# dylkot/cNMF

Measured on NVIDIA H100. Metric: NMF restarts/sec on NxG counts, K-sweep x100 seeds, 1/2/4/8 H100 vs sklearn CPU, higher is better.
Workload: dtype f32 (2-pass split-fp16 tensor-core products of group-normalised factors x exact integer counts, fp32 accumulate)

## Files before the change

cnmf_b200/_lib.py:

```python
import ctypes
import os

import numpy as np

_HERE = os.path.dirname(os.path.abspath(__file__))
LIB_PATH = os.path.join(_HERE, "libcnmf_b200.so")

SOLVER_MU, SOLVER_CD = 0, 1
PRECISION_FP32, PRECISION_TF32X3, PRECISION_TF32X3_GENERAL, PRECISION_F16X2, PRECISION_FP64 = 0, 1, 2, 3, 4
LOSS_FROBENIUS, LOSS_KULLBACK_LEIBLER, LOSS_ITAKURA_SAITO = 0, 1, 2
INIT_RANDOM, INIT_NNDSVD, INIT_NNDSVDA, INIT_NNDSVDAR = 0, 1, 2, 3
INIT_CODES = {"random": INIT_RANDOM, "nndsvd": INIT_NNDSVD, "nndsvda": INIT_NNDSVDA, "nndsvdar": INIT_NNDSVDAR}
MAX_COMPONENTS = 32


class CnmfError(RuntimeError):
    pass


class NmfParams(ctypes.Structure):
    _fields_ = [("solver", ctypes.c_int32), ("precision", ctypes.c_int32), ("max_iter", ctypes.c_int32),
                ("reserved", ctypes.c_int32), ("tol", ctypes.c_double),
                ("l1_reg_W", ctypes.c_double), ("l2_reg_W", ctypes.c_double),
                ("l1_reg_H", ctypes.c_double), ("l2_reg_H", ctypes.c_double),
                ("beta_loss", ctypes.c_int32), ("reserved2", ctypes.c_int32)]


UNIT_SOLVER_NONE = -1
UNIT_PIECES_NONE, UNIT_PIECES_TF32, UNIT_PIECES_F16 = 0, 1, 2
UNIT_GRAM_NONE, UNIT_GRAM_FUSED, UNIT_GRAM_STANDALONE = 0, 1, 2


class UpdateStepArgs(ctypes.Structure):
    _fields_ = [("n_slots", ctypes.c_int32), ("n_rids", ctypes.c_int32),
                ("ks", ctypes.c_void_p), ("rids", ctypes.c_void_p), ("done", ctypes.c_void_p),
                ("n", ctypes.c_int32), ("cpb_tiles", ctypes.c_int32), ("solver", ctypes.c_int32),
                ("pieces", ctypes.c_int32), ("gram", ctypes.c_int32), ("want_scalar", ctypes.c_int32),
                ("nsplit", ctypes.c_int32), ("l1", ctypes.c_float), ("l2", ctypes.c_float),
                ("F", ctypes.c_void_p), ("num", ctypes.c_void_p), ("gram_in", ctypes.c_void_p),
                ("piece_scale", ctypes.c_void_p), ("pieces_hi", ctypes.c_void_p), ("pieces_lo", ctypes.c_void_p),
                ("tile_scale", ctypes.c_void_p), ("gram_out", ctypes.c_void_p), ("scal_out", ctypes.c_void_p)]


UNIT_BETA_UPDATE, UNIT_BETA_DIVERGENCE = 0, 1
UNIT_SIDE_W, UNIT_SIDE_H = 0, 1


class BetaStepArgs(ctypes.Structure):
    _fields_ = [("n_slots", ctypes.c_int32), ("n_rids", ctypes.c_int32),
                ("ks", ctypes.c_void_p), ("rids", ctypes.c_void_p), ("done", ctypes.c_void_p),
                ("op", ctypes.c_int32), ("side", ctypes.c_int32), ("loss", ctypes.c_int32),
                ("n_items", ctypes.c_int32), ("n_contract", ctypes.c_int32), ("l1", ctypes.c_float), ("l2", ctypes.c_float),
                ("D", ctypes.c_void_p), ("F_own", ctypes.c_void_p), ("F_other", ctypes.c_void_p),
                ("oth_sum", ctypes.c_void_p), ("last", ctypes.c_void_p), ("totals", ctypes.c_void_p)]


_c = ctypes
_vp, _i, _ll, _d = _c.c_void_p, _c.c_int, _c.c_longlong, _c.c_double
_pp = _c.POINTER

SIGNATURES = {
    "cnmf_abi_version": (_i, []),
    "cnmf_last_error": (_c.c_char_p, []),
    "cnmf_create": (_i, [_pp(_vp), _i]),
    "cnmf_destroy": (_i, [_vp]),
    "cnmf_launch_count": (_ll, [_vp]),
    "cnmf_mem_info": (_i, [_vp, _pp(_ll), _pp(_ll), _pp(_ll)]),
    "cnmf_solve_bytes_per_row": (_ll, [_vp]),
    "cnmf_profile_enable": (_i, [_vp, _i]),
    "cnmf_profile_get": (_i, [_vp, _pp(_d), _pp(_ll), _pp(_d)]),
    "cnmf_profile_get_class": (_i, [_vp, _i, _pp(_d), _pp(_ll), _pp(_d)]),
    "cnmf_last_timing": (_i, [_vp, _pp(_d), _pp(_d), _pp(_d), _pp(_d)]),
    "cnmf_dataset_create": (_i, [_vp, _vp, _i, _i, _ll, _i, _i, _vp, _pp(_vp)]),
    "cnmf_dataset_create_csc": (_i, [_vp, _i, _i, _ll, _vp, _vp, _vp, _i, _vp, _pp(_vp)]),
    "cnmf_dataset_dense_bytes": (_i, [_i, _i, _i, _pp(_ll)]),
    "cnmf_dataset_from_columns": (_i, [_vp, _vp, _vp, _i, _vp, _pp(_vp)]),
    "cnmf_dataset_destroy": (_i, [_vp]),
    "cnmf_dataset_shape": (_i, [_vp, _pp(_i), _pp(_i)]),
    "cnmf_dataset_ld": (_i, [_vp, _pp(_i), _pp(_i)]),
    "cnmf_dataset_is_exact": (_i, [_vp]),
    "cnmf_dataset_sums": (_i, [_vp, _pp(_d), _pp(_d)]),
    "cnmf_dataset_min": (_i, [_vp, _pp(_c.c_float), _vp]),
    "cnmf_dataset_col_stats": (_i, [_vp, _vp, _vp, _vp]),
    "cnmf_dataset_row_sums": (_i, [_vp, _vp, _vp]),
    "cnmf_dataset_scaled_col_stats": (_i, [_vp, _vp, _vp, _vp, _vp]),
    "cnmf_dataset_scale_rows": (_i, [_vp, _vp, _vp, _pp(_vp)]),
    "cnmf_dataset_tpm_stats": (_i, [_vp, _d, _vp, _vp, _vp, _vp]),
    "cnmf_random_init_host": (_i, [_c.c_uint32, _d, _i, _i, _i, _vp, _ll, _vp, _ll]),
    "cnmf_random_init_dev": (_i, [_vp, _i, _vp, _vp, _vp, _vp, _vp]),
    "cnmf_nndsvd_init_dev": (_i, [_vp, _i, _vp, _vp, _i, _vp, _vp, _vp]),
    "cnmf_nndsvd_chunk_limit": (_i, [_vp, _i]),
    "cnmf_nndsvd_gemm_host": (_i, [_vp, _i, _i, _vp, _vp, _vp]),
    "cnmf_dataset_create_f64": (_i, [_vp, _vp, _i, _i, _ll, _i, _vp, _pp(_vp)]),
    "cnmf_dataset_from_columns_f64": (_i, [_vp, _vp, _vp, _i, _vp, _pp(_vp)]),
    "cnmf_factorize_f64": (_i, [_vp, _i, _vp, _vp, _pp(NmfParams), _vp, _vp, _vp, _vp, _vp]),
    "cnmf_factorize_init_f64": (_i, [_vp, _i, _vp, _vp, _vp, _pp(NmfParams), _vp, _vp, _vp, _vp, _vp]),
    "cnmf_refit_f64": (_i, [_vp, _i, _i, _vp, _pp(NmfParams), _vp, _pp(_c.c_int32), _pp(_d), _vp]),
    "cnmf_project_rows_f64": (_i, [_vp, _i, _vp, _vp, _vp]),
    "cnmf_factorize": (_i, [_vp, _i, _vp, _vp, _pp(NmfParams), _vp, _vp, _vp, _vp, _vp]),
    "cnmf_factorize_seeds_dev": (_i, [_vp, _i, _vp, _vp, _pp(NmfParams), _vp, _ll, _vp, _vp, _vp]),
    "cnmf_allgather_spectra": (_i, [_vp, _vp, _ll, _ll, _vp, _vp]),
    "cnmf_comm_unique_id": (_i, [_vp]),
    "cnmf_comm_create": (_i, [_vp, _vp, _i, _i, _pp(_vp)]),
    "cnmf_comm_destroy": (_i, [_vp]),
    "cnmf_factorize_init": (_i, [_vp, _i, _vp, _vp, _vp, _pp(NmfParams), _vp, _vp, _vp, _vp, _vp]),
    "cnmf_factorize_dev": (_i, [_vp, _i, _vp, _vp, _vp, _pp(NmfParams), _vp, _vp, _vp, _vp]),
    "cnmf_refit": (_i, [_vp, _i, _i, _vp, _pp(NmfParams), _vp, _pp(_c.c_int32), _pp(_d), _vp]),
    "cnmf_project_rows": (_i, [_vp, _i, _vp, _vp, _vp]),
    "cnmf_gemm_abt_host": (_i, [_vp, _i, _vp, _vp, _i, _i, _i, _i, _i, _vp, _vp, _vp, _i, _pp(_c.c_float), _vp]),
    "cnmf_update_step_host": (_i, [_vp, _pp(UpdateStepArgs), _vp]),
    "cnmf_beta_step_host": (_i, [_vp, _pp(BetaStepArgs), _vp]),
    "cnmf_l2_normalize_rows": (_i, [_vp, _vp, _i, _i, _i, _vp]),
    "cnmf_local_density": (_i, [_vp, _vp, _i, _i, _i, _i, _vp, _vp, _vp]),
    "cnmf_col_stats_dev": (_i, [_vp, _vp, _i, _i, _i, _vp, _vp, _vp]),
    "cnmf_gather_rows": (_i, [_vp, _vp, _i, _vp, _i, _i, _vp, _i, _vp]),
    "cnmf_sq_dists_to_rows": (_i, [_vp, _vp, _i, _i, _i, _vp, _i, _vp, _vp]),
    "cnmf_kmeans_step": (_i, [_vp, _vp, _i, _i, _i, _i, _vp, _vp, _vp, _vp, _vp, _vp, _vp, _vp, _pp(_c.c_int32), _pp(_c.c_int32), _pp(_d), _vp]),
    "cnmf_kmeans_fit": (_i, [_vp, _vp, _i, _i, _i, _i, _i, _i, _d, _vp, _vp, _i, _vp, _vp, _vp, _pp(_c.c_int32), _vp]),
    "cnmf_kmeans_assign": (_i, [_vp, _vp, _i, _i, _i, _vp, _i, _vp, _vp, _vp, _vp, _vp, _vp, _vp]),
    "cnmf_cluster_dist_sums": (_i, [_vp, _vp, _i, _i, _i, _vp, _i, _vp, _vp]),
    "cnmf_cluster_median": (_i, [_vp, _vp, _i, _i, _i, _vp, _i, _vp, _i, _vp]),
    "cnmf_l2_normalize_rows_f64": (_i, [_vp, _vp, _i, _i, _i, _vp]),
    "cnmf_local_density_f64": (_i, [_vp, _vp, _i, _i, _i, _i, _vp, _vp, _vp]),
    "cnmf_col_stats_dev_f64": (_i, [_vp, _vp, _i, _i, _i, _vp, _vp, _vp]),
    "cnmf_gather_rows_f64": (_i, [_vp, _vp, _i, _vp, _i, _i, _vp, _i, _vp]),
    "cnmf_sq_dists_to_rows_f64": (_i, [_vp, _vp, _i, _i, _i, _vp, _i, _vp, _vp]),
    "cnmf_kmeans_step_f64": (_i, [_vp, _vp, _i, _i, _i, _i, _vp, _vp, _vp, _vp, _vp, _vp, _pp(_c.c_int32), _pp(_c.c_int32), _pp(_d), _vp]),
    "cnmf_kmeans_fit_f64": (_i, [_vp, _vp, _i, _i, _i, _i, _i, _i, _d, _vp, _vp, _i, _vp, _vp, _vp, _pp(_c.c_int32), _vp]),
    "cnmf_kmeans_assign_f64": (_i, [_vp, _vp, _i, _i, _i, _vp, _i, _vp, _vp, _vp, _vp, _vp, _vp, _vp]),
    "cnmf_cluster_dist_sums_f64": (_i, [_vp, _vp, _i, _i, _i, _vp, _i, _vp, _vp]),
    "cnmf_cluster_median_f64": (_i, [_vp, _vp, _i, _i, _i, _vp, _i, _vp, _i, _vp]),
}

_lib = None


ABI_VERSION = 14


def load():
    global _lib
    if _lib is not None:
        return _lib
    if not os.path.exists(LIB_PATH):
        raise CnmfError(
            "libcnmf_b200.so not found at %s -- build it with `python -m cnmf_b200.build` "
            "(cnmf_b200 has no CPU / PyTorch fallback)" % LIB_PATH)
    lib = ctypes.CDLL(LIB_PATH)
    for name, (res, args) in SIGNATURES.items():
        fn = getattr(lib, name)
        fn.restype = res
        fn.argtypes = args
    if lib.cnmf_abi_version() != ABI_VERSION:
        raise CnmfError("libcnmf_b200.so ABI version mismatch")
    _lib = lib
    return lib


def check(rc):
    if rc != 0:
        msg = load().cnmf_last_error()
        raise CnmfError("cnmf_b200 error %d: %s" % (rc, msg.decode() if msg else "?"))


def ptr(a):
    if a is None:
        return None
    assert a.flags["C_CONTIGUOUS"]
    return a.ctypes.data_as(ctypes.c_void_p)


def f32c(a):
    return np.ascontiguousarray(a, dtype=np.float32)


def f64c(a):
    return np.ascontiguousarray(a, dtype=np.float64)
```

cnmf_b200/csrc/capi_refit.cu:

```cuda
#include <algorithm>
#include <chrono>
#include <cmath>
#include <cstring>
#include <vector>

#include "engine.h"
#include "gemm.h"
#include "nmf_kernels.cuh"

using namespace cnmf;

namespace {

__global__ void fill_kernel(float* p, float v, int rows, int n, int ld) {
  const long long total = (long long)rows * n;
  for (long long i = blockIdx.x * (long long)blockDim.x + threadIdx.x; i < total; i += (long long)gridDim.x * blockDim.x)
    p[(i / n) * ld + (i % n)] = v;
}

template <typename T>
__global__ void col_stats_kernel(const T* __restrict__ X, int rows, int cols, int ld,
                                 const double* __restrict__ row_scale, double* __restrict__ part) {
  const int c = blockIdx.x * blockDim.x + threadIdx.x;
  if (c >= cols) return;
  const int per = (rows + gridDim.y - 1) / gridDim.y;
  const int r0 = blockIdx.y * per, r1 = min(rows, r0 + per);
  double s = 0.0, q = 0.0;
  for (int r = r0; r < r1; ++r) {
    double v = X[(long long)r * ld + c];
    if (row_scale) v *= row_scale[r];
    s += v;
    q += v * v;
  }
  part[((long long)blockIdx.y * 2) * cols + c] = s;
  part[((long long)blockIdx.y * 2 + 1) * cols + c] = q;
}

__global__ void gather_cols_div_kernel(const double* __restrict__ src, int rows, int ld_src, const int* __restrict__ cols,
                                       const double* __restrict__ divisor, int n_cols, double* __restrict__ dst,
                                       int ld_dst) {
  const int c = blockIdx.x * blockDim.x + threadIdx.x;
  if (c >= n_cols) return;
  const int sc = cols[c];
  const double f = divisor[c];
  for (int r = blockIdx.y; r < rows; r += gridDim.y)
    dst[(long long)r * ld_dst + c] = __ddiv_rn(src[(long long)r * ld_src + sc], f);
}

__global__ void transpose64_kernel(const double* __restrict__ F, int k, int n, int ld, double* __restrict__ out) {
  const long long total = (long long)n * k;
  for (long long i = blockIdx.x * (long long)blockDim.x + threadIdx.x; i < total; i += (long long)gridDim.x * blockDim.x)
    out[i] = F[(i % k) * ld + i / k];
}

__global__ void col_stats_reduce_kernel(const double* __restrict__ part, int strips, int cols, double* __restrict__ out) {
  const int c = blockIdx.x * blockDim.x + threadIdx.x;
  if (c >= cols) return;
  double s = 0.0, q = 0.0;
  for (int y = 0; y < strips; ++y) {
    s += part[((long long)y * 2) * cols + c];
    q += part[((long long)y * 2 + 1) * cols + c];
  }
  out[c] = s;
  out[cols + c] = q;
}

__global__ void row_sums_kernel(const float* __restrict__ X, int rows, int cols, int ld, double* __restrict__ out) {
  const int r = (blockIdx.x * blockDim.x + threadIdx.x) >> 5, lane = threadIdx.x & 31;
  if (r >= rows) return;
  const float* row = X + (long long)r * ld;
  double s = 0.0;
  for (int c = lane; c < cols; c += 32) s += (double)row[c];
  s = warp_sum(s);
  if (lane == 0) out[r] = s;
}

__global__ void scale_rows_kernel(const float* __restrict__ src, int rows, int cols, int ld, const float* __restrict__ rs,
                                  float* __restrict__ dst) {
  const long long total = (long long)rows * (ld / 4);
  for (long long i = blockIdx.x * (long long)blockDim.x + threadIdx.x; i < total; i += (long long)gridDim.x * blockDim.x) {
    const int r = (int)(i / (ld / 4));
    float4 v = reinterpret_cast<const float4*>(src)[i];
    const float f = rs[r];
    v.x *= f; v.y *= f; v.z *= f; v.w *= f;
    reinterpret_cast<float4*>(dst)[i] = v;
  }
}

__global__ void combine_scale_kernel(const float* __restrict__ scale, const float* __restrict__ src_cs,
                                     const int* __restrict__ cols, int n, int n_pad, float* __restrict__ out) {
  const int c = blockIdx.x * blockDim.x + threadIdx.x;
  if (c >= n_pad) return;
  out[c] = (c < n) ? scale[c] * (src_cs ? src_cs[cols[c]] : 1.f) : 0.f;
}

__global__ void gather_cols_kernel(const float* __restrict__ src, int rows, int ld_src, const int* __restrict__ cols,
                                   const float* __restrict__ scale, int n_cols, float* __restrict__ dst, int ld_dst) {
  const int c = blockIdx.x * blockDim.x + threadIdx.x;
  if (c >= n_cols) return;
  const int sc = cols[c];
  const float f = scale[c];
  for (int r = blockIdx.y; r < rows; r += gridDim.y) dst[(long long)r * ld_dst + c] = src[(long long)r * ld_src + sc] * f;
}

}

extern "C" {

static void finish_col_stats(double n, int n_cols, double* mean_host, double* var_host) {
  for (int c = 0; c < n_cols; ++c) {
    const double m = mean_host[c] / n;
    mean_host[c] = m;
    var_host[c] = std::max(var_host[c] / n - m * m, 0.0);
  }
}

static int col_stats_impl(cnmf_dataset_t d, const double* row_scale_host, double* mean_host, double* var_host, void* stream) {
  CNMF_REQUIRE(d && mean_host && var_host, "col_stats: NULL argument");
  cnmf_handle_s* h = d->h;
  cudaStream_t s = as_stream(stream);
  CNMF_CUDA_CHECK(cudaSetDevice(h->device));
  if (row_scale_host) CNMF_TRY(require_dense(d, "scaled_col_stats"));
  const bool f64 = d->precision == CNMF_PRECISION_FP64;
  double* buf = d->col_sums;
  if (!d->sparse) {
    const int strips = std::max(1, std::min(64, d->n_rows / 64));
    double* part = static_cast<double*>(h->dev_buf("colstats.part", sizeof(double) * 2 * (size_t)strips * d->n_cols));
    buf = static_cast<double*>(h->dev_buf("colstats", sizeof(double) * 2 * d->n_cols));
    double* d_rs = nullptr;
    if (row_scale_host) {
      d_rs = static_cast<double*>(h->dev_buf("colstats.rs", sizeof(double) * d->n_rows));
      if (!d_rs) return -2;
      CNMF_CUDA_CHECK(cudaMemcpyAsync(d_rs, row_scale_host, sizeof(double) * d->n_rows, cudaMemcpyHostToDevice, s));
    }
    if (!part || !buf) return -2;
    dim3 grid((d->n_cols + 127) / 128, strips);
    if (f64) col_stats_kernel<<<grid, 128, 0, s>>>(d->X64, d->n_rows, d->n_cols, d->ld_c, d_rs, part);
    else col_stats_kernel<<<grid, 128, 0, s>>>(d->X, d->n_rows, d->n_cols, d->ld_c, d_rs, part);
    col_stats_reduce_kernel<<<(d->n_cols + 127) / 128, 128, 0, s>>>(part, strips, d->n_cols, buf);
    CNMF_CUDA_CHECK(cudaGetLastError());
    h->launches += 2;
  }
  CNMF_CUDA_CHECK(cudaMemcpyAsync(mean_host, buf, sizeof(double) * d->n_cols, cudaMemcpyDeviceToHost, s));
  CNMF_CUDA_CHECK(cudaMemcpyAsync(var_host, buf + d->n_cols, sizeof(double) * d->n_cols, cudaMemcpyDeviceToHost, s));
  CNMF_CUDA_CHECK(cudaStreamSynchronize(s));
  finish_col_stats(d->n_rows, d->n_cols, mean_host, var_host);
  return 0;
}

int cnmf_dataset_col_stats(cnmf_dataset_t d, double* mean_host, double* var_host, void* stream) {
  return col_stats_impl(d, nullptr, mean_host, var_host, stream);
}

int cnmf_dataset_scaled_col_stats(cnmf_dataset_t d, const double* row_scale_host, double* mean_host, double* var_host,
                                  void* stream) {
  CNMF_REQUIRE(row_scale_host, "scaled_col_stats: NULL row scale");
  return col_stats_impl(d, row_scale_host, mean_host, var_host, stream);
}

int cnmf_dataset_row_sums(cnmf_dataset_t d, double* row_sums_host, void* stream) {
  CNMF_REQUIRE(d && row_sums_host, "row_sums: NULL argument");
  CNMF_TRY(require_dense(d, "row_sums"));
  cnmf_handle_s* h = d->h;
  cudaStream_t s = as_stream(stream);
  CNMF_CUDA_CHECK(cudaSetDevice(h->device));
  double* buf = static_cast<double*>(h->dev_buf("rowsums", sizeof(double) * d->n_rows));
  if (!buf) return -2;
  row_sums_kernel<<<(d->n_rows + 7) / 8, 256, 0, s>>>(d->X, d->n_rows, d->n_cols, d->ld_c, buf);
  CNMF_CUDA_CHECK(cudaGetLastError());
  h->launches += 1;
  CNMF_CUDA_CHECK(cudaMemcpyAsync(row_sums_host, buf, sizeof(double) * d->n_rows, cudaMemcpyDeviceToHost, s));
  CNMF_CUDA_CHECK(cudaStreamSynchronize(s));
  return 0;
}

int cnmf_dataset_tpm_stats(cnmf_dataset_t d, double target_sum, double* totals_host, double* mean_host,
                           double* var_host, void* stream) {
  CNMF_REQUIRE(d && totals_host && mean_host && var_host, "tpm_stats: NULL argument");
  if (!d->sparse) {
    set_last_error("tpm_stats is implemented for sparse (CSC) datasets only: a dense dataset gives the same numbers "
                   "through row_sums and scaled_col_stats");
    return -3;
  }
  cnmf_handle_s* h = d->h;
  cudaStream_t s = as_stream(stream);
  CNMF_CUDA_CHECK(cudaSetDevice(h->device));
  double* tot = static_cast<double*>(h->dev_buf("rowsums", sizeof(double) * d->n_rows));
  double* sums = static_cast<double*>(h->dev_buf("colstats", sizeof(double) * 2 * d->n_cols));
  if (!tot || !sums) return -2;
  CNMF_TRY(csc_tpm_sums(d, target_sum, tot, sums, s));
  CNMF_CUDA_CHECK(cudaMemcpyAsync(totals_host, tot, sizeof(double) * d->n_rows, cudaMemcpyDeviceToHost, s));
  CNMF_CUDA_CHECK(cudaMemcpyAsync(mean_host, sums, sizeof(double) * d->n_cols, cudaMemcpyDeviceToHost, s));
  CNMF_CUDA_CHECK(cudaMemcpyAsync(var_host, sums + d->n_cols, sizeof(double) * d->n_cols, cudaMemcpyDeviceToHost, s));
  CNMF_CUDA_CHECK(cudaStreamSynchronize(s));
  finish_col_stats(d->n_rows, d->n_cols, mean_host, var_host);
  return 0;
}

int cnmf_dataset_from_columns(cnmf_dataset_t src, const int32_t* cols_host, const float* col_scale_host, int n_cols,
                              void* stream, cnmf_dataset_t* out) {
  CNMF_REQUIRE(src && cols_host && col_scale_host && out && n_cols > 0, "dataset_from_columns: bad arguments");
  CNMF_TRY(require_f32(src, "dataset_from_columns"));
  for (int c = 0; c < n_cols; ++c)
    CNMF_REQUIRE(cols_host[c] >= 0 && cols_host[c] < src->n_cols, "dataset_from_columns: column index out of range");
  cnmf_handle_s* h = src->h;
  cudaStream_t s = as_stream(stream);
  CNMF_CUDA_CHECK(cudaSetDevice(h->device));
  int* d_cols = static_cast<int*>(h->dev_buf("fromcols.idx", sizeof(int) * n_cols));
  float* d_scale = static_cast<float*>(h->dev_buf("fromcols.scale", sizeof(float) * n_cols));
  if (!d_cols || !d_scale) return -2;
  CNMF_CUDA_CHECK(cudaMemcpyAsync(d_cols, cols_host, sizeof(int) * n_cols, cudaMemcpyHostToDevice, s));
  CNMF_CUDA_CHECK(cudaMemcpyAsync(d_scale, col_scale_host, sizeof(float) * n_cols, cudaMemcpyHostToDevice, s));
  auto* d = new cnmf_dataset_s(h, src->n_rows, n_cols, src->precision);
  int rc = dataset_alloc(d, &d->X, (size_t)d->n_rows * d->ld_c);
  if (rc == 0) {
    cudaError_t e = cudaMemsetAsync(d->X, 0, (size_t)d->n_rows * d->ld_c * sizeof(float), s);
    if (e != cudaSuccess) rc = -2;
  }
  if (rc == 0 && src->sparse) {
    rc = csc_gather_cols(src, d_cols, d_scale, n_cols, d->X, d->ld_c, s);
  } else if (rc == 0) {
    dim3 grid((n_cols + 127) / 128, std::min(d->n_rows, 16384));
    gather_cols_kernel<<<grid, 128, 0, s>>>(src->X, d->n_rows, src->ld_c, d_cols, d_scale, n_cols, d->X, d->ld_c);
    h->launches += 1;
    if (cudaGetLastError() != cudaSuccess) rc = -2;
  }
  const bool exact = form_exact(src->form);
  if (rc == 0 && exact) {
    rc = dataset_alloc(d, &d->col_scale, (size_t)d->ld_c);
    if (rc == 0) {
      combine_scale_kernel<<<(d->ld_c + 255) / 256, 256, 0, s>>>(d_scale, src->col_scale, d_cols, n_cols, d->ld_c, d->col_scale);
      h->launches += 1;
      if (cudaGetLastError() != cudaSuccess) rc = -2;
    }
    if (rc == 0 && src->row_scale) {
      rc = dataset_alloc(d, &d->row_scale, (size_t)d->ld_r);
      if (rc == 0 && cudaMemcpyAsync(d->row_scale, src->row_scale, sizeof(float) * d->ld_r, cudaMemcpyDeviceToDevice, s) != cudaSuccess)
        rc = -2;
    }
  }
  if (rc == 0) rc = dataset_finish(d, s, exact);
  if (rc != 0) {
    cnmf_dataset_destroy(d);
    return rc;
  }
  *out = d;
  return 0;
}

int cnmf_dataset_scale_rows(cnmf_dataset_t src, const float* row_scale_host, void* stream, cnmf_dataset_t* out) {
  CNMF_REQUIRE(src && row_scale_host && out, "dataset_scale_rows: bad arguments");
  CNMF_TRY(require_dense(src, "scale_rows"));
  cnmf_handle_s* h = src->h;
  cudaStream_t s = as_stream(stream);
  CNMF_CUDA_CHECK(cudaSetDevice(h->device));
  float* d_rs = static_cast<float*>(h->dev_buf("scalerows.rs", sizeof(float) * src->n_rows));
  if (!d_rs) return -2;
  CNMF_CUDA_CHECK(cudaMemcpyAsync(d_rs, row_scale_host, sizeof(float) * src->n_rows, cudaMemcpyHostToDevice, s));
  auto* d = new cnmf_dataset_s(h, src->n_rows, src->n_cols, src->precision);
  int rc = dataset_alloc(d, &d->X, (size_t)d->n_rows * d->ld_c);
  if (rc == 0) {
    scale_rows_kernel<<<NUM_SMS * 8, 256, 0, s>>>(src->X, d->n_rows, d->n_cols, d->ld_c, d_rs, d->X);
    h->launches += 1;
    if (cudaGetLastError() != cudaSuccess) rc = -2;
  }
  if (rc == 0) rc = dataset_finish(d, s);
  if (rc != 0) {
    cnmf_dataset_destroy(d);
    return rc;
  }
  *out = d;
  return 0;
}

int cnmf_refit(cnmf_dataset_t d, int transposed, int k, const float* fixed_host, const cnmf_nmf_params* p,
               float* out_host, int32_t* n_iter_host, double* err_host, void* stream) {
  CNMF_REQUIRE(d && fixed_host && p && out_host, "refit: NULL argument");
  CNMF_TRY(require_f32(d, "refit"));
  CNMF_TRY(check_params_precision(d, p));
  CNMF_REQUIRE(k >= 1 && k <= KMAX, "refit: n_components must be in [1, 32] on the CUDA path");
  if (d->sparse && !transposed) CNMF_TRY(require_dense(d, "refit with transposed = 0"));
  if (d->sparse && p->beta_loss != CNMF_LOSS_FROBENIUS) CNMF_TRY(require_dense(d, "refit with a KL / IS beta_loss"));
  const auto t_enter = std::chrono::steady_clock::now();
  cnmf_handle_s* h = d->h;
  cudaStream_t s = as_stream(stream);
  CNMF_CUDA_CHECK(cudaSetDevice(h->device));
  if (p->beta_loss != CNMF_LOSS_FROBENIUS) CNMF_TRY(dataset_ensure_full_transpose(d, s));
  const DataView v = make_view(d, transposed != 0);

  const size_t nr = (size_t)k * v.ld_r, nc = (size_t)k * v.ld_c;
  float* Fr = static_cast<float*>(h->dev_buf("refit.Fr", nr * 4));
  float* Fc = static_cast<float*>(h->dev_buf("refit.Fc", nc * 4));
  if (!Fr || !Fc) return -2;
  CNMF_CUDA_CHECK(cudaMemsetAsync(Fr, 0, nr * 4, s));
  CNMF_CUDA_CHECK(cudaMemsetAsync(Fc, 0, nc * 4, s));
  CNMF_CUDA_CHECK(cudaMemcpy2DAsync(Fc, (size_t)v.ld_c * 4, fixed_host, (size_t)v.n_c * 4, (size_t)v.n_c * 4, k,
                                    cudaMemcpyHostToDevice, s));
  if (p->solver == CNMF_SOLVER_MU) {
    const double mean = v.sum / ((double)v.n_r * (double)v.n_c);
    fill_kernel<<<NUM_SMS * 4, 256, 0, s>>>(Fr, (float)std::sqrt(mean / k), k, v.n_r, v.ld_r);
    CNMF_CUDA_CHECK(cudaGetLastError());
    h->launches += 1;
  }
  SolveIO io;
  io.R = 1;
  io.ks = {k};
  io.Fr = Fr;
  io.Fc = Fc;
  io.update_cols = false;
  if (d->sparse) {
    const int kp = round_up(k, 4);
    float* U = static_cast<float*>(h->dev_buf("refit.U", (size_t)v.n_c * kp * 4));
    float* NUM = static_cast<float*>(h->dev_buf("refit.NUM", nr * 4));
    if (!U || !NUM) return -2;
    CNMF_CUDA_CHECK(cudaMemsetAsync(NUM, 0, nr * 4, s));
    CNMF_TRY(stage_rows(h, Fc, k, v.n_c, v.ld_c, kp, U, s));
    CNMF_TRY(csc_project(d, U, k, kp, NUM, v.ld_r, s));
    io.num_rows = NUM;
  }
  auto t_solve = std::chrono::steady_clock::now();
  if (h->profile) {
    CNMF_CUDA_CHECK(cudaStreamSynchronize(s));
    h->t_h2d_ms = std::chrono::duration<double, std::milli>(t_solve - t_enter).count();
    t_solve = std::chrono::steady_clock::now();
  }
  CNMF_TRY(solve_batched(h, v, io, *p, s));
  if (h->profile) h->t_solve_ms = std::chrono::duration<double, std::milli>(std::chrono::steady_clock::now() - t_solve).count();

  float* T = static_cast<float*>(h->dev_buf("refit.T", (size_t)v.n_r * k * 4));
  float* T_host = static_cast<float*>(h->host_buf("refit.T_host", (size_t)v.n_r * k * 4));
  if (!T || !T_host) return -2;
  CNMF_TRY(launch_transpose(Fr, k, v.n_r, v.ld_r, T, nullptr, nullptr, k, s));
  h->launches += 1;
  CNMF_CUDA_CHECK(cudaMemcpyAsync(T_host, T, (size_t)v.n_r * k * 4, cudaMemcpyDeviceToHost, s));
  CNMF_CUDA_CHECK(cudaStreamSynchronize(s));
  std::memcpy(out_host, T_host, (size_t)v.n_r * k * 4);
  if (n_iter_host) *n_iter_host = io.n_iter[0];
  if (err_host) *err_host = io.err[0];
  return 0;
}

int cnmf_project_rows(cnmf_dataset_t d, int k, const float* Ut_host, float* out_host, void* stream) {
  CNMF_REQUIRE(d && Ut_host && out_host && k >= 1, "project_rows: bad arguments");
  CNMF_TRY(require_f32(d, "project_rows"));
  cnmf_handle_s* h = d->h;
  cudaStream_t s = as_stream(stream);
  CNMF_CUDA_CHECK(cudaSetDevice(h->device));
  if (d->sparse) {
    CNMF_REQUIRE(k <= KMAX, "project_rows: k must be <= 32 on a sparse dataset");
    const int kp = round_up(k, 4);
    float* Ut = static_cast<float*>(h->dev_buf("proj.Ut", (size_t)k * d->n_rows * 4));
    float* U = static_cast<float*>(h->dev_buf("proj.U", (size_t)d->n_rows * kp * 4));
    float* C = static_cast<float*>(h->dev_buf("proj.C", (size_t)k * d->ld_c * 4));
    if (!Ut || !U || !C) return -2;
    CNMF_CUDA_CHECK(cudaMemcpyAsync(Ut, Ut_host, (size_t)k * d->n_rows * 4, cudaMemcpyHostToDevice, s));
    CNMF_TRY(stage_rows(h, Ut, k, d->n_rows, d->n_rows, kp, U, s));
    CNMF_TRY(csc_project(d, U, k, kp, C, d->ld_c, s));
    CNMF_CUDA_CHECK(cudaMemcpy2DAsync(out_host, (size_t)d->n_cols * 4, C, (size_t)d->ld_c * 4, (size_t)d->n_cols * 4, k,
                                      cudaMemcpyDeviceToHost, s));
    CNMF_CUDA_CHECK(cudaStreamSynchronize(s));
    return 0;
  }
  const DataView v = make_view(d, false);
  const size_t nr = (size_t)k * d->ld_r;
  float* A = static_cast<float*>(h->dev_buf("proj.A", nr * 4));
  float *A_hi = nullptr, *A_lo = nullptr, *A_rs = nullptr;
  if (!A) return -2;
  CNMF_CUDA_CHECK(cudaMemsetAsync(A, 0, nr * 4, s));
  CNMF_CUDA_CHECK(cudaMemcpy2DAsync(A, (size_t)d->ld_r * 4, Ut_host, (size_t)d->n_rows * 4, (size_t)d->n_rows * 4, k,
                                    cudaMemcpyHostToDevice, s));
  if (v.form != Form::FP32) {
    A_hi = static_cast<float*>(h->dev_buf("proj.A_hi", nr * 4));
    A_lo = static_cast<float*>(h->dev_buf("proj.A_lo", nr * 4));
    if (!A_hi || !A_lo) return -2;
    if (v.form == Form::F16_EXACT) {
      A_rs = static_cast<float*>(h->dev_buf("proj.A_rs", sizeof(float) * (size_t)k * ((d->ld_r + 511) / 512)));
      if (!A_rs) return -2;
    }
    CNMF_TRY(make_pieces(v.form, A, k, d->n_rows, d->ld_r, v.scale_r, A_hi, A_lo, A_rs, s));
    h->launches += 1;
  }
  GemmArgs g{};
  g.M = k; g.N = d->n_cols; g.Kd = d->n_rows;
  g.lda = d->ld_r; g.ldb = d->ld_r; g.ldc = d->ld_c;
  int splits = 1;
  {
    const int tiles = ((k + 127) / 128) * ((d->n_cols + 255) / 256);
    if (tiles < 2 * h->sm_count) splits = (2 * h->sm_count + tiles - 1) / tiles;
    splits = std::min(splits, std::max(1, ((d->n_rows + 31) / 32) / 8));
    splits = std::min(splits, 32);
    splits = gemm_effective_splits(d->n_rows, splits, v.form == Form::F16_EXACT ? 1 : 0);
  }
  g.splits = g.splits_effective = splits;
  g.c_split_stride = (long long)k * d->ld_c;
  float* C = static_cast<float*>(h->dev_buf("proj.C", (size_t)splits * k * d->ld_c * 4));
  if (!C) return -2;
  g.C = C;
  CNMF_TRY(form_gemm(v.form, g, A, A_hi, A_lo, A_rs, v.B_cols, v.scale_c, s));
  h->launches += 1;
  std::vector<float> tmp((size_t)splits * k * d->ld_c);
  CNMF_CUDA_CHECK(cudaMemcpyAsync(tmp.data(), C, tmp.size() * 4, cudaMemcpyDeviceToHost, s));
  CNMF_CUDA_CHECK(cudaStreamSynchronize(s));
  for (int c = 0; c < k; ++c)
    for (int j = 0; j < d->n_cols; ++j) {
      double a = 0.0;
      for (int z = 0; z < splits; ++z) a += tmp[(size_t)z * k * d->ld_c + (size_t)c * d->ld_c + j];
      out_host[(size_t)c * d->n_cols + j] = (float)a;
    }
  return 0;
}

int cnmf_dataset_from_columns_f64(cnmf_dataset_t src, const int32_t* cols_host, const double* divisor_host, int n_cols,
                                  void* stream, cnmf_dataset_t* out) {
  CNMF_REQUIRE(src && cols_host && divisor_host && out && n_cols > 0, "dataset_from_columns_f64: bad arguments");
  CNMF_TRY(require_f64(src, "dataset_from_columns"));
  for (int c = 0; c < n_cols; ++c)
    CNMF_REQUIRE(cols_host[c] >= 0 && cols_host[c] < src->n_cols, "dataset_from_columns_f64: column index out of range");
  cnmf_handle_s* h = src->h;
  cudaStream_t s = as_stream(stream);
  CNMF_CUDA_CHECK(cudaSetDevice(h->device));
  int* d_cols = static_cast<int*>(h->dev_buf("fromcols.idx", sizeof(int) * n_cols));
  double* d_div = static_cast<double*>(h->dev_buf("fromcols.div64", sizeof(double) * n_cols));
  if (!d_cols || !d_div) return -2;
  CNMF_CUDA_CHECK(cudaMemcpyAsync(d_cols, cols_host, sizeof(int) * n_cols, cudaMemcpyHostToDevice, s));
  CNMF_CUDA_CHECK(cudaMemcpyAsync(d_div, divisor_host, sizeof(double) * n_cols, cudaMemcpyHostToDevice, s));
  auto* d = new cnmf_dataset_s(h, src->n_rows, n_cols, CNMF_PRECISION_FP64);
  d->form = Form::FP64;
  const size_t nx = (size_t)d->n_rows * d->ld_c;
  float* buf = nullptr;
  int rc = dataset_alloc(d, &buf, 2 * nx);
  if (rc == 0) {
    d->X64 = reinterpret_cast<double*>(buf);
    if (cudaMemsetAsync(d->X64, 0, nx * sizeof(double), s) != cudaSuccess) rc = -2;
  }
  if (rc == 0) {
    dim3 grid((n_cols + 127) / 128, std::min(d->n_rows, 16384));
    gather_cols_div_kernel<<<grid, 128, 0, s>>>(src->X64, d->n_rows, src->ld_c, d_cols, d_div, n_cols, d->X64, d->ld_c);
    h->launches += 1;
    if (cudaGetLastError() != cudaSuccess) rc = -2;
  }
  double sums[2] = {0.0, 0.0};
  if (rc == 0) rc = matrix_sums_f64(h, d->X64, d->n_rows, d->n_cols, d->ld_c, sums, s);
  if (rc != 0) {
    cnmf_dataset_destroy(d);
    return rc;
  }
  d->sum = sums[0];
  d->sum_sq = sums[1];
  *out = d;
  return 0;
}

int cnmf_refit_f64(cnmf_dataset_t d, int transposed, int k, const double* fixed_host, const cnmf_nmf_params* p,
                   double* out_host, int32_t* n_iter_host, double* err_host, void* stream) {
  CNMF_REQUIRE(d && fixed_host && p && out_host, "refit_f64: NULL argument");
  CNMF_TRY(require_f64(d, "refit"));
  CNMF_TRY(check_params_precision(d, p));
  CNMF_REQUIRE(k >= 1 && k <= KMAX, "refit_f64: n_components must be in [1, 32] on the CUDA path");
  if (p->beta_loss != CNMF_LOSS_FROBENIUS) {
    set_last_error("cnmf_refit_f64: float64 datasets support beta_loss = frobenius only");
    return -3;
  }
  cnmf_handle_s* h = d->h;
  cudaStream_t s = as_stream(stream);
  CNMF_CUDA_CHECK(cudaSetDevice(h->device));
  const DataView v = make_view(d, transposed != 0);
  const size_t nr = (size_t)k * v.ld_r, nc = (size_t)k * v.ld_c;
  double* Fr = static_cast<double*>(h->dev_buf("refit.Fr64", nr * 8));
  double* Fc = static_cast<double*>(h->dev_buf("refit.Fc64", nc * 8));
  double* T = static_cast<double*>(h->dev_buf("refit.T64", (size_t)v.n_r * k * 8));
  if (!Fr || !Fc || !T) return -2;
  CNMF_CUDA_CHECK(cudaMemsetAsync(Fr, 0, nr * 8, s));
  CNMF_CUDA_CHECK(cudaMemsetAsync(Fc, 0, nc * 8, s));
  CNMF_CUDA_CHECK(cudaMemcpy2DAsync(Fc, (size_t)v.ld_c * 8, fixed_host, (size_t)v.n_c * 8, (size_t)v.n_c * 8, k,
                                    cudaMemcpyHostToDevice, s));
  if (p->solver == CNMF_SOLVER_MU) {
    const double mean = v.sum / ((double)v.n_r * (double)v.n_c);
    CNMF_TRY(fill_f64(Fr, std::sqrt(mean / k), k, v.n_r, v.ld_r, s));
    h->launches += 1;
  }
  SolveIO io;
  io.R = 1;
  io.ks = {k};
  io.Fr64 = Fr;
  io.Fc64 = Fc;
  io.update_cols = false;
  CNMF_TRY(solve_batched(h, v, io, *p, s));
  transpose64_kernel<<<NUM_SMS * 4, 256, 0, s>>>(Fr, k, v.n_r, v.ld_r, T);
  CNMF_CUDA_CHECK(cudaGetLastError());
  h->launches += 1;
  CNMF_CUDA_CHECK(cudaMemcpyAsync(out_host, T, (size_t)v.n_r * k * 8, cudaMemcpyDeviceToHost, s));
  CNMF_CUDA_CHECK(cudaStreamSynchronize(s));
  if (n_iter_host) *n_iter_host = io.n_iter[0];
  if (err_host) *err_host = io.err[0];
  return 0;
}

int cnmf_project_rows_f64(cnmf_dataset_t d, int k, const double* Ut_host, double* out_host, void* stream) {
  CNMF_REQUIRE(d && Ut_host && out_host && k >= 1, "project_rows_f64: bad arguments");
  CNMF_TRY(require_f64(d, "project_rows"));
  cnmf_handle_s* h = d->h;
  cudaStream_t s = as_stream(stream);
  CNMF_CUDA_CHECK(cudaSetDevice(h->device));
  const size_t na = (size_t)k * d->ld_r, nc = (size_t)k * d->ld_c;
  double* A = static_cast<double*>(h->dev_buf("proj.A64", na * 8));
  double* C = static_cast<double*>(h->dev_buf("proj.C64", nc * 8));
  if (!A || !C) return -2;
  CNMF_CUDA_CHECK(cudaMemsetAsync(A, 0, na * 8, s));
  CNMF_CUDA_CHECK(cudaMemcpy2DAsync(A, (size_t)d->ld_r * 8, Ut_host, (size_t)d->n_rows * 8, (size_t)d->n_rows * 8, k,
                                    cudaMemcpyHostToDevice, s));
  h->launches += 1;
  CNMF_TRY(launch_gemm_f64(A, d->ld_r, k, d->X64, d->n_rows, d->n_cols, d->ld_c, true, C, d->ld_c, s));
  CNMF_CUDA_CHECK(cudaMemcpy2DAsync(out_host, (size_t)d->n_cols * 8, C, (size_t)d->ld_c * 8, (size_t)d->n_cols * 8, k,
                                    cudaMemcpyDeviceToHost, s));
  CNMF_CUDA_CHECK(cudaStreamSynchronize(s));
  return 0;
}

int cnmf_gemm_abt_host(cnmf_handle_t h, int precision, const float* A, const float* B, int M, int N, int Kd, int splits,
                       int b_exact, const float* k_scale, const float* out_col_scale, float* C, int reps, float* ms_out,
                       void* stream) {
  CNMF_REQUIRE(h && A && B && C && M > 0 && N > 0 && Kd > 0, "gemm_abt_host: bad arguments");
  const bool f16 = precision == CNMF_PRECISION_F16X2;
  CNMF_REQUIRE(!b_exact || f16 || precision == CNMF_PRECISION_TF32X3, "gemm_abt_host: b_exact needs tf32x3 or f16x2");
  const bool exact = f16 || b_exact;
  CNMF_REQUIRE(exact || (!k_scale && !out_col_scale), "gemm_abt_host: k_scale / out_col_scale need an exact form");
  const Form form = f16 ? Form::F16_EXACT
                  : precision != CNMF_PRECISION_TF32X3 ? Form::FP32
                  : b_exact ? Form::TF32_EXACT : Form::TF32;
  cudaStream_t s = as_stream(stream);
  CNMF_CUDA_CHECK(cudaSetDevice(h->device));
  const int lda = pad_ld(Kd), ldc = pad_ld(N);
  const size_t na = (size_t)M * lda, nb = (size_t)N * lda;
  float* dA = static_cast<float*>(h->dev_buf("gemmtest.A", na * 4));
  float* dB = static_cast<float*>(h->dev_buf("gemmtest.B", nb * 4));
  float* dAh = static_cast<float*>(h->dev_buf("gemmtest.Ah", na * 4));
  float* dAl = static_cast<float*>(h->dev_buf("gemmtest.Al", na * 4));
  float* dBh = static_cast<float*>(h->dev_buf("gemmtest.Bh", nb * 4));
  float* dBl = static_cast<float*>(h->dev_buf("gemmtest.Bl", nb * 4));
  const int se = gemm_effective_splits(Kd, splits, f16 ? 1 : 0);
  float* dC = static_cast<float*>(h->dev_buf("gemmtest.C", (size_t)se * M * ldc * 4));
  float* dRs = static_cast<float*>(h->dev_buf("gemmtest.rs", sizeof(float) * (size_t)M * ((lda + 511) / 512)));
  if (!dA || !dB || !dAh || !dAl || !dBh || !dBl || !dC || !dRs) return -2;
  CNMF_CUDA_CHECK(cudaMemsetAsync(dA, 0, na * 4, s));
  CNMF_CUDA_CHECK(cudaMemsetAsync(dB, 0, nb * 4, s));
  CNMF_CUDA_CHECK(cudaMemcpy2DAsync(dA, (size_t)lda * 4, A, (size_t)Kd * 4, (size_t)Kd * 4, M, cudaMemcpyHostToDevice, s));
  CNMF_CUDA_CHECK(cudaMemcpy2DAsync(dB, (size_t)lda * 4, B, (size_t)Kd * 4, (size_t)Kd * 4, N, cudaMemcpyHostToDevice, s));
  float* dKs = nullptr;
  float* dCs = nullptr;
  if (k_scale) {
    dKs = static_cast<float*>(h->dev_buf("gemmtest.kscale", (size_t)lda * 4));
    if (!dKs) return -2;
    CNMF_CUDA_CHECK(cudaMemsetAsync(dKs, 0, (size_t)lda * 4, s));
    CNMF_CUDA_CHECK(cudaMemcpyAsync(dKs, k_scale, (size_t)Kd * 4, cudaMemcpyHostToDevice, s));
  }
  if (out_col_scale) {
    dCs = static_cast<float*>(h->dev_buf("gemmtest.cscale", (size_t)ldc * 4));
    if (!dCs) return -2;
    CNMF_CUDA_CHECK(cudaMemsetAsync(dCs, 0, (size_t)ldc * 4, s));
    CNMF_CUDA_CHECK(cudaMemcpyAsync(dCs, out_col_scale, (size_t)N * 4, cudaMemcpyHostToDevice, s));
  }
  if (f16) CNMF_TRY(launch_to_half(dB, dBh, (long long)nb, s));
  else if (form != Form::FP32) CNMF_TRY(launch_split_tf32(dB, dBh, dBl, (long long)nb, s));
  CNMF_TRY(make_pieces(form, dA, M, Kd, lda, dKs, dAh, dAl, dRs, s));
  CNMF_CUDA_CHECK(cudaMemsetAsync(dC, 0xff, (size_t)se * M * ldc * 4, s));
  GemmArgs g{};
  g.M = M; g.N = N; g.Kd = Kd; g.lda = lda; g.ldb = lda; g.ldc = ldc;
  g.C = dC; g.c_split_stride = (long long)M * ldc; g.splits = splits; g.splits_effective = se;
  const Operand Bop{dB, dBh, dBl, N, Kd, lda};
  cudaEvent_t e0, e1;
  CNMF_CUDA_CHECK(cudaEventCreate(&e0));
  CNMF_CUDA_CHECK(cudaEventCreate(&e1));
  if (reps < 1) reps = 1;
  int rc = form_gemm(form, g, dA, dAh, dAl, dRs, Bop, dCs, s);
  if (rc == 0 && reps > 1) {
    cudaEventRecord(e0, s);
    for (int i = 0; i < reps && rc == 0; ++i) rc = form_gemm(form, g, dA, dAh, dAl, dRs, Bop, dCs, s);
    cudaEventRecord(e1, s);
  }
  h->launches += reps;
  if (rc != 0) return rc;
  std::vector<float> tmp((size_t)se * M * ldc);
  CNMF_CUDA_CHECK(cudaMemcpyAsync(tmp.data(), dC, tmp.size() * 4, cudaMemcpyDeviceToHost, s));
  CNMF_CUDA_CHECK(cudaStreamSynchronize(s));
  if (ms_out) {
    float ms = 0.f;
    if (reps > 1) cudaEventElapsedTime(&ms, e0, e1);
    *ms_out = reps > 1 ? ms / reps : 0.f;
  }
  cudaEventDestroy(e0);
  cudaEventDestroy(e1);
  for (int m = 0; m < M; ++m)
    for (int n = 0; n < N; ++n) {
      double a = 0.0;
      for (int z = 0; z < se; ++z) a += tmp[(size_t)z * M * ldc + (size_t)m * ldc + n];
      C[(size_t)m * N + n] = (float)a;
    }
  return 0;
}

}
```

cnmf_b200/csrc/gemm.h:

```cpp
#pragma once
#include <cuda_runtime.h>

namespace cnmf {

struct GemmArgs {
  const float* A_hi;
  const float* A_lo;
  const float* B_hi;
  const float* B_lo;
  float* C;
  int M, N, Kd;
  int lda, ldb, ldc;
  long long c_split_stride;
  int splits;
  int splits_effective;
  int b_exact;
  const float* out_col_scale;
  int f16;
  const float* a_tile_scale;
  int a_tiles;
};

int gemm_effective_splits(int Kd, int splits, int f16 = 0);

int gemm_fixed_splits(int Kd, int f16 = 0);

int gemm_tf32x3(const GemmArgs& g, cudaStream_t stream);

int gemm_fp32_simt(const GemmArgs& g, cudaStream_t stream);

}
```

cnmf_b200/csrc/gemm_tf32x3.cu:

```cuda
#include <cuda.h>
#include <cuda_runtime.h>
#include <cstdint>
#include <cstdio>
#include <algorithm>
#include <map>
#include <mutex>
#include <tuple>

#include "common.cuh"
#include "gemm.h"

namespace cnmf {

namespace {

constexpr int BN = 128;
constexpr int BK = 32;
constexpr long long WAIT_TIMEOUT_CYCLES = 4000000000LL;

template <int BM>
constexpr int num_threads() { return 128 * (1 + BM / 64); }

template <int BM, int STAGES, bool BEXACT>
struct SmemLayout {
  static constexpr int A_BYTES = BM * BK * 4;
  static constexpr int B_BYTES = BN * BK * 4;
  static constexpr int STAGE_BYTES = 2 * A_BYTES + (BEXACT ? 1 : 2) * B_BYTES;
  static constexpr int BAR_OFFSET = STAGES * STAGE_BYTES;
  static constexpr int TOTAL = BAR_OFFSET + 3 * STAGES * 8;
  static constexpr int DYN_BYTES = TOTAL + 1024;
  static_assert(DYN_BYTES <= 227 * 1024, "pipeline stages do not fit the shared memory of an SM");
};

__device__ __forceinline__ void mbar_init(uint32_t bar, uint32_t count) {
  asm volatile("mbarrier.init.shared::cta.b64 [%0], %1;" ::"r"(bar), "r"(count) : "memory");
}
__device__ __forceinline__ void mbar_arrive_expect_tx(uint32_t bar, uint32_t bytes) {
  asm volatile("mbarrier.arrive.expect_tx.shared::cta.b64 _, [%0], %1;" ::"r"(bar), "r"(bytes) : "memory");
}
__device__ __forceinline__ void mbar_arrive(uint32_t bar) {
  asm volatile("mbarrier.arrive.shared::cta.b64 _, [%0];" ::"r"(bar) : "memory");
}
__device__ __forceinline__ bool mbar_try_wait(uint32_t bar, uint32_t parity) {
  uint32_t ok;
  asm volatile(
      "{\n\t.reg .pred p;\n\t"
      "mbarrier.try_wait.parity.shared::cta.b64 p, [%1], %2;\n\t"
      "selp.u32 %0, 1, 0, p;\n\t}"
      : "=r"(ok)
      : "r"(bar), "r"(parity)
      : "memory");
  return ok != 0;
}
template <bool TRAP>
__device__ __forceinline__ void mbar_wait(uint32_t bar, uint32_t parity) {
  if (mbar_try_wait(bar, parity)) return;
  const long long t0 = clock64();
  while (!mbar_try_wait(bar, parity)) {
    if (TRAP && clock64() - t0 > WAIT_TIMEOUT_CYCLES) __trap();
  }
}
__device__ __forceinline__ void tma_load_2d(uint32_t dst, const CUtensorMap* map, uint32_t bar, int c0, int c1) {
  asm volatile(
      "cp.async.bulk.tensor.2d.shared::cluster.global.mbarrier::complete_tx::bytes [%0], [%1, {%3, %4}], [%2];"
      ::"r"(dst), "l"(reinterpret_cast<uint64_t>(map)), "r"(bar), "r"(c0), "r"(c1)
      : "memory");
}
__device__ __forceinline__ void tma_load_2d_multicast(uint32_t dst, const CUtensorMap* map, uint32_t bar, int c0, int c1,
                                                      uint16_t mask) {
  asm volatile(
      "cp.async.bulk.tensor.2d.shared::cluster.global.mbarrier::complete_tx::bytes.multicast::cluster"
      " [%0], [%1, {%3, %4}], [%2], %5;"
      ::"r"(dst), "l"(reinterpret_cast<uint64_t>(map)), "r"(bar), "r"(c0), "r"(c1), "h"(mask)
      : "memory");
}

__device__ __forceinline__ void mbar_arrive_remote(uint32_t bar, uint32_t rank) {
  asm volatile(
      "{\n\t.reg .b32 remote;\n\t"
      "mapa.shared::cluster.u32 remote, %0, %1;\n\t"
      "mbarrier.arrive.shared::cluster.b64 _, [remote];\n\t}"
      ::"r"(bar), "r"(rank)
      : "memory");
}
__device__ __forceinline__ void cluster_sync() {
  asm volatile("barrier.cluster.arrive.release;\n\tbarrier.cluster.wait.acquire;" ::: "memory");
}

__device__ __forceinline__ uint64_t make_smem_desc(uint32_t smem_addr) {
  uint64_t d = 0;
  d |= static_cast<uint64_t>((smem_addr & 0x3FFFFu) >> 4);
  d |= static_cast<uint64_t>(1) << 16;
  d |= static_cast<uint64_t>(1024 >> 4) << 32;
  d |= static_cast<uint64_t>(1) << 62;
  return d;
}

__device__ __forceinline__ void named_bar_sync(uint32_t id, uint32_t count) {
  asm volatile("bar.sync %0, %1;" ::"r"(id), "r"(count) : "memory");
}
__device__ __forceinline__ void named_bar_arrive(uint32_t id, uint32_t count) {
  asm volatile("bar.arrive %0, %1;" ::"r"(id), "r"(count) : "memory");
}

template <int N>
__device__ __forceinline__ void setmaxnreg_dec() { asm volatile("setmaxnreg.dec.sync.aligned.u32 %0;" ::"n"(N)); }
template <int N>
__device__ __forceinline__ void setmaxnreg_inc() { asm volatile("setmaxnreg.inc.sync.aligned.u32 %0;" ::"n"(N)); }

__device__ __forceinline__ void wgmma_fence() { asm volatile("wgmma.fence.sync.aligned;" ::: "memory"); }
__device__ __forceinline__ void wgmma_commit() { asm volatile("wgmma.commit_group.sync.aligned;" ::: "memory"); }
template <int N>
__device__ __forceinline__ void wgmma_wait() { asm volatile("wgmma.wait_group.sync.aligned %0;" ::"n"(N) : "memory"); }

template <bool F16>
__device__ __forceinline__ void wgmma_m64n128(float (&d)[64], uint64_t adesc, uint64_t bdesc, uint32_t acc) {
  if constexpr (F16) {
    asm volatile(
      "{\n\t.reg .pred p;\n\t"
      "setp.ne.b32 p, %66, 0;\n\t"
      "wgmma.mma_async.sync.aligned.m64n128k16.f32.f16.f16 {"
      "%0, %1, %2, %3, %4, %5, %6, %7, %8, %9, %10, %11, %12, %13, %14, %15, "
      "%16, %17, %18, %19, %20, %21, %22, %23, %24, %25, %26, %27, %28, %29, %30, %31, "
      "%32, %33, %34, %35, %36, %37, %38, %39, %40, %41, %42, %43, %44, %45, %46, %47, "
      "%48, %49, %50, %51, %52, %53, %54, %55, %56, %57, %58, %59, %60, %61, %62, %63 "
      "}, %64, %65, p, 1, 1, 0, 0;\n\t}"
      : "+f"(d[0]), "+f"(d[1]), "+f"(d[2]), "+f"(d[3]), "+f"(d[4]), "+f"(d[5]), "+f"(d[6]), "+f"(d[7]),
        "+f"(d[8]), "+f"(d[9]), "+f"(d[10]), "+f"(d[11]), "+f"(d[12]), "+f"(d[13]), "+f"(d[14]), "+f"(d[15]),
        "+f"(d[16]), "+f"(d[17]), "+f"(d[18]), "+f"(d[19]), "+f"(d[20]), "+f"(d[21]), "+f"(d[22]), "+f"(d[23]),
        "+f"(d[24]), "+f"(d[25]), "+f"(d[26]), "+f"(d[27]), "+f"(d[28]), "+f"(d[29]), "+f"(d[30]), "+f"(d[31]),
        "+f"(d[32]), "+f"(d[33]), "+f"(d[34]), "+f"(d[35]), "+f"(d[36]), "+f"(d[37]), "+f"(d[38]), "+f"(d[39]),
        "+f"(d[40]), "+f"(d[41]), "+f"(d[42]), "+f"(d[43]), "+f"(d[44]), "+f"(d[45]), "+f"(d[46]), "+f"(d[47]),
        "+f"(d[48]), "+f"(d[49]), "+f"(d[50]), "+f"(d[51]), "+f"(d[52]), "+f"(d[53]), "+f"(d[54]), "+f"(d[55]),
        "+f"(d[56]), "+f"(d[57]), "+f"(d[58]), "+f"(d[59]), "+f"(d[60]), "+f"(d[61]), "+f"(d[62]), "+f"(d[63])
      : "l"(adesc), "l"(bdesc), "r"(acc));
  } else {
    asm volatile(
      "{\n\t.reg .pred p;\n\t"
      "setp.ne.b32 p, %66, 0;\n\t"
      "wgmma.mma_async.sync.aligned.m64n128k8.f32.tf32.tf32 {"
      "%0, %1, %2, %3, %4, %5, %6, %7, %8, %9, %10, %11, %12, %13, %14, %15, "
      "%16, %17, %18, %19, %20, %21, %22, %23, %24, %25, %26, %27, %28, %29, %30, %31, "
      "%32, %33, %34, %35, %36, %37, %38, %39, %40, %41, %42, %43, %44, %45, %46, %47, "
      "%48, %49, %50, %51, %52, %53, %54, %55, %56, %57, %58, %59, %60, %61, %62, %63 "
      "}, %64, %65, p, 1, 1;\n\t}"
      : "+f"(d[0]), "+f"(d[1]), "+f"(d[2]), "+f"(d[3]), "+f"(d[4]), "+f"(d[5]), "+f"(d[6]), "+f"(d[7]),
        "+f"(d[8]), "+f"(d[9]), "+f"(d[10]), "+f"(d[11]), "+f"(d[12]), "+f"(d[13]), "+f"(d[14]), "+f"(d[15]),
        "+f"(d[16]), "+f"(d[17]), "+f"(d[18]), "+f"(d[19]), "+f"(d[20]), "+f"(d[21]), "+f"(d[22]), "+f"(d[23]),
        "+f"(d[24]), "+f"(d[25]), "+f"(d[26]), "+f"(d[27]), "+f"(d[28]), "+f"(d[29]), "+f"(d[30]), "+f"(d[31]),
        "+f"(d[32]), "+f"(d[33]), "+f"(d[34]), "+f"(d[35]), "+f"(d[36]), "+f"(d[37]), "+f"(d[38]), "+f"(d[39]),
        "+f"(d[40]), "+f"(d[41]), "+f"(d[42]), "+f"(d[43]), "+f"(d[44]), "+f"(d[45]), "+f"(d[46]), "+f"(d[47]),
        "+f"(d[48]), "+f"(d[49]), "+f"(d[50]), "+f"(d[51]), "+f"(d[52]), "+f"(d[53]), "+f"(d[54]), "+f"(d[55]),
        "+f"(d[56]), "+f"(d[57]), "+f"(d[58]), "+f"(d[59]), "+f"(d[60]), "+f"(d[61]), "+f"(d[62]), "+f"(d[63])
      : "l"(adesc), "l"(bdesc), "r"(acc));
  }
}

struct TileOrder {
  int m_tiles, n_pairs, group, group_n;
};

__host__ __device__ __forceinline__ void decode_item(int w, const TileOrder& o, int& mt, int& np, int& z) {
  const int per_slice = o.m_tiles * o.n_pairs;
  z = w / per_slice;
  int r = w - z * per_slice;
  const int q_tiles = o.group_n ? o.n_pairs : o.m_tiles;
  const int p_tiles = o.group_n ? o.m_tiles : o.n_pairs;
  const int g0 = r / (o.group * p_tiles) * o.group;
  r -= g0 * p_tiles;
  const int gq = q_tiles - g0 < o.group ? q_tiles - g0 : o.group;
  const int p = r / gq, q = g0 + r % gq;
  mt = o.group_n ? p : q;
  np = o.group_n ? q : p;
}

template <int BM, int STAGES, bool BEXACT, bool F16>
__device__ __forceinline__ void
gemm_body(const CUtensorMap& tmA_hi, const CUtensorMap& tmA_lo, const CUtensorMap& tmB_hi, const CUtensorMap& tmB_lo,
          float* __restrict__ C, int M, int ldc, long long c_split_stride,
          const TileOrder& ord, int n_tiles, int splits, int total_kb, int kb_per_split, int chain_kb,
          const float* __restrict__ out_scale, const float* __restrict__ a_tile_scale, int a_tiles, int a_gshift) {
  static_assert(!F16 || BEXACT, "the fp16 path exists for exact integer B operands only");
  static_assert(BM == 128 || BM == 192, "two or three consumer warpgroups");
  constexpr int NC = BM / 64;
  constexpr int BKE = F16 ? 2 * BK : BK;
  constexpr int KSTEP_BYTES = 32;
  using L = SmemLayout<BM, STAGES, BEXACT>;
  extern __shared__ uint8_t smem_raw[];
  const uint32_t smem_base = (smem_u32(smem_raw) + 1023u) & ~1023u;

  const uint32_t bar_base = smem_base + L::BAR_OFFSET;
  auto full_bar = [&](int s) { return bar_base + 8u * s; };
  auto empty_bar = [&](int s) { return bar_base + 8u * (STAGES + s); };
  auto peer_free_bar = [&](int s) { return bar_base + 8u * (2 * STAGES + s); };

  const int wg = __shfl_sync(0xffffffffu, static_cast<int>(threadIdx.x >> 7), 0);
  const int warp = (threadIdx.x >> 5) & 3;
  const int lane = threadIdx.x & 31;
  const int rank = blockIdx.x & 1, cluster = blockIdx.x >> 1, clusters = gridDim.x >> 1;

  if (threadIdx.x == 0) {
    for (int s = 0; s < STAGES; ++s) {
      mbar_init(full_bar(s), 1);
      mbar_init(empty_bar(s), 4 * NC);
      mbar_init(peer_free_bar(s), 1);
    }
    asm volatile("fence.mbarrier_init.release.cluster;" ::: "memory");
  }
  cluster_sync();

  const int items = ord.m_tiles * ord.n_pairs * splits;

  constexpr bool REBALANCE = NC == 3;
  if (wg == 0) {
    if constexpr (REBALANCE) setmaxnreg_dec<32>();
    if (threadIdx.x == 0) {
      int stage = 0;
      uint32_t phase = 0;
      constexpr uint32_t stage_tx = static_cast<uint32_t>(L::STAGE_BYTES);
      constexpr uint32_t HALF_A = L::A_BYTES / 2;
      for (int w = cluster; w < items; w += clusters) {
        int mt, np, z;
        decode_item(w, ord, mt, np, z);
        const int nt = 2 * np + rank;
        const int kb0 = z * kb_per_split;
        const int kb1 = min(total_kb, kb0 + kb_per_split);
        for (int kb = kb0; kb < kb1; ++kb) {
          mbar_wait<true>(empty_bar(stage), phase ^ 1u);
          mbar_arrive_remote(peer_free_bar(stage), rank ^ 1);
          mbar_wait<true>(peer_free_bar(stage), phase);
          const uint32_t st = smem_base + stage * L::STAGE_BYTES;
          mbar_arrive_expect_tx(full_bar(stage), stage_tx);
          tma_load_2d_multicast(st + rank * HALF_A, &tmA_hi, full_bar(stage), kb * BKE, mt * BM + rank * (BM / 2), 0x3);
          tma_load_2d_multicast(st + L::A_BYTES + rank * HALF_A, &tmA_lo, full_bar(stage), kb * BKE,
                                mt * BM + rank * (BM / 2), 0x3);
          tma_load_2d(st + 2 * L::A_BYTES, &tmB_hi, full_bar(stage), kb * BKE, nt * BN);
          if constexpr (!BEXACT) tma_load_2d(st + 2 * L::A_BYTES + L::B_BYTES, &tmB_lo, full_bar(stage), kb * BKE, nt * BN);
          if (++stage == STAGES) { stage = 0; phase ^= 1u; }
        }
      }
      for (int s = 0; s < STAGES; ++s) {
        mbar_wait<true>(empty_bar(stage), phase ^ 1u);
        if (++stage == STAGES) { stage = 0; phase ^= 1u; }
      }
    }
  } else {
    if constexpr (REBALANCE) setmaxnreg_inc<160>();
    constexpr uint32_t TURN_BAR = 1, TURN_THREADS = 256;
    const int cw = wg - 1;
    const uint32_t a_off = static_cast<uint32_t>(cw * 64 * 128);
    const uint32_t next_bar = TURN_BAR + (cw + 1 == NC ? 0 : cw + 1);
    if (cw == NC - 1) named_bar_arrive(TURN_BAR, TURN_THREADS);
    int stage = 0;
    uint32_t phase = 0;
    for (int w = cluster; w < items; w += clusters) {
      int mt, np, z;
      decode_item(w, ord, mt, np, z);
      const int nt = 2 * np + rank;
      const int kb0 = z * kb_per_split;
      const int kb1 = min(total_kb, kb0 + kb_per_split);
      const int row0 = mt * BM + cw * 64 + warp * 16 + (lane >> 2);
      float acc[64];
#pragma unroll
      for (int i = 0; i < 64; ++i) acc[i] = 0.f;
      const float* sc_row0 = (F16 && a_tile_scale && row0 < M) ? a_tile_scale + static_cast<long long>(row0) * a_tiles : nullptr;
      const float* sc_row1 = (F16 && a_tile_scale && row0 + 8 < M) ? a_tile_scale + static_cast<long long>(row0 + 8) * a_tiles : nullptr;
      for (int c0 = kb0; c0 < kb1; c0 += chain_kb) {
        const int c1 = min(kb1, c0 + chain_kb);
        float d[64];
        int prev = -1;
        for (int kb = c0; kb < c1; ++kb) {
          mbar_wait<false>(full_bar(stage), phase);
          named_bar_sync(TURN_BAR + cw, TURN_THREADS);
          const uint32_t st = smem_base + stage * L::STAGE_BYTES;
          const uint64_t a_hi = make_smem_desc(st + a_off);
          const uint64_t a_lo = make_smem_desc(st + L::A_BYTES + a_off);
          const uint64_t b_hi = make_smem_desc(st + 2 * L::A_BYTES);
          const uint64_t b_lo = make_smem_desc(st + 2 * L::A_BYTES + L::B_BYTES);
          wgmma_fence();
#pragma unroll
          for (int k = 0; k < BK * 4 / KSTEP_BYTES; ++k) {
            const uint64_t koff = static_cast<uint64_t>((k * KSTEP_BYTES) >> 4);
            const uint32_t acc0 = (kb > c0 || k > 0) ? 1u : 0u;
            wgmma_m64n128<F16>(d, a_lo + koff, b_hi + koff, acc0);
            if constexpr (!BEXACT) wgmma_m64n128<F16>(d, a_hi + koff, b_lo + koff, 1u);
            wgmma_m64n128<F16>(d, a_hi + koff, b_hi + koff, 1u);
          }
          wgmma_commit();
          named_bar_arrive(next_bar, TURN_THREADS);
          if (prev >= 0) {
            wgmma_wait<1>();
            if (lane == 0) mbar_arrive(empty_bar(prev));
          }
          prev = stage;
          if (++stage == STAGES) { stage = 0; phase ^= 1u; }
        }
        wgmma_wait<0>();
        if (lane == 0) mbar_arrive(empty_bar(prev));
        if constexpr (F16) {
          const float s0 = sc_row0 ? sc_row0[c0 >> a_gshift] : 1.f;
          const float s1 = sc_row1 ? sc_row1[c0 >> a_gshift] : 1.f;
#pragma unroll
          for (int i = 0; i < 64; i += 4) {
            acc[i] = fmaf(d[i], s0, acc[i]);
            acc[i + 1] = fmaf(d[i + 1], s0, acc[i + 1]);
            acc[i + 2] = fmaf(d[i + 2], s1, acc[i + 2]);
            acc[i + 3] = fmaf(d[i + 3], s1, acc[i + 3]);
          }
        } else {
#pragma unroll
          for (int i = 0; i < 64; ++i) acc[i] += d[i];
        }
      }
      if (nt >= n_tiles) continue;
      constexpr int EPI_J = 8;
      float* cbase = C + static_cast<long long>(z) * c_split_stride;
      const int colq = nt * BN + 2 * (lane & 3);
#pragma unroll
      for (int j0 = 0; j0 < 16; j0 += EPI_J) {
        float2 sc[EPI_J];
#pragma unroll
        for (int j = 0; j < EPI_J; ++j) {
          const int col = colq + 8 * (j0 + j);
          sc[j] = out_scale && col < ldc ? *reinterpret_cast<const float2*>(out_scale + col) : make_float2(1.f, 1.f);
        }
#pragma unroll
        for (int j = 0; j < EPI_J; ++j) {
          const int col = colq + 8 * (j0 + j);
          if (col >= ldc) continue;
          const float* a = acc + 4 * (j0 + j);
          if (row0 < M)
            *reinterpret_cast<float2*>(cbase + static_cast<long long>(row0) * ldc + col) =
                make_float2(a[0] * sc[j].x, a[1] * sc[j].y);
          if (row0 + 8 < M)
            *reinterpret_cast<float2*>(cbase + static_cast<long long>(row0 + 8) * ldc + col) =
                make_float2(a[2] * sc[j].x, a[3] * sc[j].y);
        }
      }
    }
    if (cw == 0) named_bar_sync(TURN_BAR, TURN_THREADS);
  }
  cluster_sync();
}

template <int BM, int STAGES, bool BEXACT, bool F16>
__global__ void __cluster_dims__(2, 1, 1) __launch_bounds__(num_threads<BM>(), 1)
gemm_tf32x3_kernel(const __grid_constant__ CUtensorMap tmA_hi, const __grid_constant__ CUtensorMap tmA_lo,
                   const __grid_constant__ CUtensorMap tmB_hi, const __grid_constant__ CUtensorMap tmB_lo,
                   float* __restrict__ C, int M, int ldc, long long c_split_stride,
                   const TileOrder ord, int n_tiles, int splits, int total_kb, int kb_per_split, int chain_kb,
                   const float* __restrict__ out_scale, const float* __restrict__ a_tile_scale, int a_tiles, int a_gshift) {
  gemm_body<BM, STAGES, BEXACT, F16>(tmA_hi, tmA_lo, tmB_hi, tmB_lo, C, M, ldc, c_split_stride, ord, n_tiles, splits,
                                     total_kb, kb_per_split, chain_kb, out_scale, a_tile_scale, a_tiles, a_gshift);
}

typedef CUresult (*PFN_encodeTiled)(CUtensorMap*, CUtensorMapDataType, cuuint32_t, void*, const cuuint64_t*,
                                    const cuuint64_t*, const cuuint32_t*, const cuuint32_t*, CUtensorMapInterleave,
                                    CUtensorMapSwizzle, CUtensorMapL2promotion, CUtensorMapFloatOOBfill);

PFN_encodeTiled get_encode_fn() {
  static PFN_encodeTiled fn = nullptr;
  static std::once_flag once;
  std::call_once(once, [] {
    void* p = nullptr;
    cudaDriverEntryPointQueryResult qres;
    if (cudaGetDriverEntryPoint("cuTensorMapEncodeTiled", &p, cudaEnableDefault, &qres) == cudaSuccess &&
        qres == cudaDriverEntryPointSuccess)
      fn = reinterpret_cast<PFN_encodeTiled>(p);
  });
  return fn;
}

struct MapKey {
  const void* ptr; int rows, cols, ld, box_rows, f16;
  bool operator<(const MapKey& o) const {
    return std::tie(ptr, rows, cols, ld, box_rows, f16) < std::tie(o.ptr, o.rows, o.cols, o.ld, o.box_rows, o.f16);
  }
};

int make_map(CUtensorMap* map, const float* ptr, int rows, int cols, int ld, int box_rows, bool f16 = false) {
  static std::mutex mu;
  static std::map<MapKey, CUtensorMap> cache;
  const MapKey key{ptr, rows, cols, ld, box_rows, f16 ? 1 : 0};
  {
    std::lock_guard<std::mutex> lock(mu);
    auto it = cache.find(key);
    if (it != cache.end()) { *map = it->second; return 0; }
  }
  PFN_encodeTiled enc = get_encode_fn();
  if (!enc) { set_last_error("cuTensorMapEncodeTiled entry point not available"); return -2; }
  const int esize = f16 ? 2 : 4;
  cuuint64_t dims[2] = {static_cast<cuuint64_t>(cols), static_cast<cuuint64_t>(rows)};
  cuuint64_t strides[1] = {static_cast<cuuint64_t>(ld) * esize};
  cuuint32_t box[2] = {static_cast<cuuint32_t>(128 / esize), static_cast<cuuint32_t>(box_rows)};
  cuuint32_t estr[2] = {1, 1};
  CUresult r = enc(map, f16 ? CU_TENSOR_MAP_DATA_TYPE_FLOAT16 : CU_TENSOR_MAP_DATA_TYPE_FLOAT32, 2, const_cast<float*>(ptr), dims, strides, box, estr,
                   CU_TENSOR_MAP_INTERLEAVE_NONE, CU_TENSOR_MAP_SWIZZLE_128B, CU_TENSOR_MAP_L2_PROMOTION_L2_256B,
                   CU_TENSOR_MAP_FLOAT_OOB_FILL_NONE);
  if (r != CUDA_SUCCESS) {
    set_last_error("cuTensorMapEncodeTiled failed with CUresult " + std::to_string(static_cast<int>(r)));
    return -2;
  }
  std::lock_guard<std::mutex> lock(mu);
  if (cache.size() >= 512) cache.clear();
  cache.emplace(key, *map);
  return 0;
}

static double order_bytes(int q_tiles, int p_tiles, double q_panel, double p_panel, int group, int grid, double budget) {
  const long long waves = (static_cast<long long>(group) * p_tiles + grid - 1) / grid;
  const double q_reads = group * q_panel <= budget ? 1.0 : static_cast<double>(std::min<long long>(p_tiles, waves));
  return q_tiles * q_panel * q_reads + static_cast<double>((q_tiles + group - 1) / group) * p_tiles * p_panel;
}

static TileOrder pick_tile_order(int m_tiles, int n_pairs, double a_panel, double b_panel, int grid, long long l2_bytes) {
  const double budget = 0.5 * static_cast<double>(l2_bytes);
  TileOrder best{m_tiles, n_pairs, m_tiles, 0};
  double best_bytes = order_bytes(m_tiles, n_pairs, a_panel, b_panel, m_tiles, grid, budget);
  for (int gn = 0; gn < 2; ++gn) {
    const int q = gn ? n_pairs : m_tiles, p = gn ? m_tiles : n_pairs;
    const double qb = gn ? b_panel : a_panel, pb = gn ? a_panel : b_panel;
    int prev = 0;
    for (int ng = 1; ng <= q; ++ng) {
      const int g = (q + ng - 1) / ng;
      if (g == prev) continue;
      prev = g;
      const double b = order_bytes(q, p, qb, pb, g, grid, budget);
      if (b < best_bytes) { best_bytes = b; best = TileOrder{m_tiles, n_pairs, g, gn}; }
    }
  }
  return best;
}

template <int BM, int STAGES, bool BEXACT, bool F16>
int launch(const GemmArgs& g, cudaStream_t stream) {
  using L = SmemLayout<BM, STAGES, BEXACT>;
  constexpr int NUM_THREADS = num_threads<BM>();
  constexpr int BKE = F16 ? 2 * BK : BK;
  CUtensorMap mAh, mAl, mBh, mBl;
  int rc;
  if ((rc = make_map(&mAh, g.A_hi, g.M, g.Kd, g.lda, BM / 2, F16))) return rc;
  if ((rc = make_map(&mAl, g.A_lo, g.M, g.Kd, g.lda, BM / 2, F16))) return rc;
  if ((rc = make_map(&mBh, g.B_hi, g.N, g.Kd, g.ldb, BN, F16))) return rc;
  if ((rc = make_map(&mBl, BEXACT ? g.B_hi : g.B_lo, g.N, g.Kd, g.ldb, BN, F16))) return rc;
  int dev = 0, l2 = 0;
  CNMF_CUDA_CHECK(cudaGetDevice(&dev));
  CNMF_CUDA_CHECK(cudaDeviceGetAttribute(&l2, cudaDevAttrL2CacheSize, dev));
  const int m_tiles = (g.M + BM - 1) / BM;
  const int n_tiles = (g.N + BN - 1) / BN;
  const int n_pairs = (n_tiles + 1) / 2;
  const int total_kb = (g.Kd + BKE - 1) / BKE;
  int splits = g.splits < 1 ? 1 : g.splits;
  if (splits > total_kb) splits = total_kb;
  int kb_per_split = (total_kb + splits - 1) / splits;
  if (F16 && (kb_per_split & 1)) ++kb_per_split;
  splits = (total_kb + kb_per_split - 1) / kb_per_split;
  if (splits != g.splits_effective) { set_last_error("gemm: splits_effective mismatch (use gemm_effective_splits)"); return -1; }

  auto kern = gemm_tf32x3_kernel<BM, STAGES, BEXACT, F16>;
  static int max_clusters[64] = {};
  int clusters_cap = dev >= 0 && dev < 64 ? max_clusters[dev] : 0;
  if (clusters_cap == 0) {
    CNMF_CUDA_CHECK(cudaFuncSetAttribute(kern, cudaFuncAttributeMaxDynamicSharedMemorySize, L::DYN_BYTES));
    cudaLaunchConfig_t cfg = {};
    cfg.gridDim = dim3(2, 1, 1);
    cfg.blockDim = dim3(NUM_THREADS, 1, 1);
    cfg.dynamicSmemBytes = L::DYN_BYTES;
    CNMF_CUDA_CHECK(cudaOccupancyMaxActiveClusters(&clusters_cap, kern, &cfg));
    if (clusters_cap < 1) { set_last_error("gemm: no 2-CTA cluster of this kernel fits the device"); return -1; }
    if (dev >= 0 && dev < 64) max_clusters[dev] = clusters_cap;
  }
  const int items = m_tiles * n_pairs * splits;
  const int clusters = items < clusters_cap ? items : clusters_cap;
  const double kslice_row = static_cast<double>(kb_per_split) * BK * 4;
  const TileOrder ord = pick_tile_order(m_tiles, n_pairs, BM * kslice_row * 2, 2 * BN * kslice_row * (BEXACT ? 1 : 2),
                                        clusters, l2);
  kern<<<2 * clusters, NUM_THREADS, L::DYN_BYTES, stream>>>(mAh, mAl, mBh, mBl, g.C, g.M, g.ldc, g.c_split_stride,
                                                            ord, n_tiles, splits, total_kb, kb_per_split, BEXACT ? 2 : 1,
                                                    g.out_col_scale, g.a_tile_scale, g.a_tiles, 3);
  CNMF_CUDA_CHECK(cudaGetLastError());
  return 0;
}

}

int gemm_fixed_splits(int Kd, int f16) {
  const int bke = f16 ? 2 * BK : BK;
  const int total_kb = (Kd + bke - 1) / bke;
  const int s = std::max(1, std::min(16, (total_kb + 63) / 64));
  return gemm_effective_splits(Kd, s, f16);
}

int gemm_effective_splits(int Kd, int splits, int f16) {
  const int bke = f16 ? 2 * BK : BK;
  const int total_kb = (Kd + bke - 1) / bke;
  if (splits < 1) splits = 1;
  if (splits > total_kb) splits = total_kb;
  int kb_per_split = (total_kb + splits - 1) / splits;
  if (f16 && (kb_per_split & 1)) ++kb_per_split;
  return (total_kb + kb_per_split - 1) / kb_per_split;
}

int gemm_tf32x3(const GemmArgs& g, cudaStream_t stream) {
  CNMF_REQUIRE(g.M > 0 && g.N > 0 && g.Kd > 0, "gemm: empty problem");
  CNMF_REQUIRE(g.lda % 4 == 0 && g.ldb % 4 == 0 && g.ldc % 4 == 0, "gemm: leading dimensions must be multiples of 4 floats");
  CNMF_REQUIRE((reinterpret_cast<uintptr_t>(g.A_hi) | reinterpret_cast<uintptr_t>(g.A_lo) |
                reinterpret_cast<uintptr_t>(g.B_hi) | reinterpret_cast<uintptr_t>(g.B_lo) |
                reinterpret_cast<uintptr_t>(g.C) | reinterpret_cast<uintptr_t>(g.out_col_scale)) % 16 == 0,
               "gemm: pointers must be 16-byte aligned");
  const bool tall = g.splits_effective > 1 && g.M >= 2048;
  if (g.f16) {
    CNMF_REQUIRE(g.b_exact, "gemm: the fp16 path needs an exact B operand");
    CNMF_REQUIRE(g.lda % 8 == 0 && g.ldb % 8 == 0, "gemm: fp16 leading dimensions must be multiples of 8 halves");
    CNMF_REQUIRE(!g.a_tile_scale || g.a_tiles * 512 >= g.Kd, "gemm: a_tiles does not cover the reduction length");
    return tall ? launch<192, 3, true, true>(g, stream) : launch<128, 4, true, true>(g, stream);
  }
  if (g.b_exact) return tall ? launch<192, 3, true, false>(g, stream) : launch<128, 4, true, false>(g, stream);
  return launch<128, 3, false, false>(g, stream);
}

}
```

cnmf_b200/engine.py:

```python
import ctypes

import numpy as np

from . import _lib
from ._lib import (LOSS_FROBENIUS, LOSS_ITAKURA_SAITO, LOSS_KULLBACK_LEIBLER, NmfParams, PRECISION_FP32,
                   PRECISION_F16X2, PRECISION_FP64, PRECISION_TF32X3, PRECISION_TF32X3_GENERAL, SOLVER_CD, SOLVER_MU,
                   check, f32c, f64c, ptr)

_DEFAULT_PRECISION = PRECISION_F16X2


def precision_code(p):
    if p in (PRECISION_FP32, PRECISION_TF32X3, PRECISION_TF32X3_GENERAL, PRECISION_F16X2, PRECISION_FP64):
        return p
    return {"fp32": PRECISION_FP32, "tf32x3": PRECISION_TF32X3, "tf32x3-general": PRECISION_TF32X3_GENERAL,
            "f16x2": PRECISION_F16X2, "fp64": PRECISION_FP64}[p]


def is_fp64(precision):
    return precision is not None and precision_code(precision) == PRECISION_FP64


def check_fp64_supported(precision, beta_loss="frobenius", rng="device"):
    if not is_fp64(precision):
        return
    if loss_code(beta_loss) != LOSS_FROBENIUS:
        raise NotImplementedError("cnmf_b200: precision='fp64' supports beta_loss='frobenius' only (got %r)"
                                  % (beta_loss,))
    if rng == "host":
        raise NotImplementedError("cnmf_b200: precision='fp64' draws its random starts on the device; rng='host' "
                                  "serves the float precisions only")


def _params_precision(p):
    return PRECISION_TF32X3 if p in (PRECISION_TF32X3_GENERAL, PRECISION_F16X2) else p


def check_supported(ks=None, init="random", beta_loss="frobenius"):
    from .nndsvd import INITS
    if ks is not None:
        bad = [int(k) for k in np.atleast_1d(ks) if int(k) < 1 or int(k) > _lib.MAX_COMPONENTS]
        if bad:
            raise ValueError("cnmf_b200: n_components must be in [1, %d] on the CUDA path (got %s); the batched "
                             "kernels keep a restart's K x K Gram matrix and its K factor values per item on chip"
                             % (_lib.MAX_COMPONENTS, bad))
    if init is not None and init not in INITS:
        raise ValueError("Invalid init parameter: got %r instead of one of %r" % (init, (None,) + INITS))
    loss_code(beta_loss)


def init_code(init, ks, n_samples, n_features):
    from .nndsvd import resolve_init
    which = {resolve_init(init, int(k), n_samples, n_features) for k in np.atleast_1d(ks)}
    if len(which) > 1:
        raise ValueError("init=%r resolves to %s for different n_components of one call; split the call by K"
                         % (init, sorted(which)))
    return _lib.INIT_CODES[which.pop()]


def nndsvd_starts(X, ks, seeds, init, dtype=np.float32):
    import concurrent.futures
    import os
    from .nndsvd import nndsvd_init, resolve_init
    ks = [int(k) for k in ks]
    n, g = X.shape
    offs = np.concatenate([[0], np.cumsum(ks)]).astype(np.int64)
    W0 = np.empty((int(offs[-1]), n), dtype)
    H0 = np.empty((int(offs[-1]), g), dtype)

    def one(r):
        which = resolve_init(init, ks[r], n, g)
        if which == "random":
            raise ValueError("init=None resolves to 'random' for n_components > min(shape): use the seeded device generator")
        W, H = nndsvd_init(X, ks[r], int(seeds[r]), which)
        W0[offs[r]:offs[r + 1]] = W.T
        H0[offs[r]:offs[r + 1]] = H

    workers = max(1, min(8, (os.cpu_count() or 1) // 4, len(ks)))
    if workers == 1:
        for r in range(len(ks)):
            one(r)
    else:
        with concurrent.futures.ThreadPoolExecutor(max_workers=workers) as ex:
            list(ex.map(one, range(len(ks))))
    return W0, H0


def make_params(nmf_kwargs, n_samples, n_features, precision, for_refit=False):
    solver = nmf_kwargs.get("solver", "mu")
    beta = nmf_kwargs.get("beta_loss", "frobenius")
    loss = loss_code(beta)
    if loss != LOSS_FROBENIUS and solver != "mu":
        raise ValueError("Invalid beta_loss parameter: solver %r does not handle beta_loss = %r" % (solver, beta))
    if not for_refit:
        check_supported(None, nmf_kwargs.get("init", "random"), beta)
    if solver not in ("mu", "cd"):
        raise ValueError("solver must be 'mu' or 'cd'")
    alpha_W = float(nmf_kwargs.get("alpha_W", 0.0))
    alpha_H = nmf_kwargs.get("alpha_H", 0.0)
    alpha_H = alpha_W if alpha_H == "same" else float(alpha_H)
    l1_ratio = float(nmf_kwargs.get("l1_ratio", 0.0))
    p = NmfParams()
    p.solver = SOLVER_MU if solver == "mu" else SOLVER_CD
    p.precision = _params_precision(precision_code(precision))
    rng = nmf_kwargs.get("rng", "device")
    if rng not in ("device", "host"):
        raise ValueError("rng must be 'device' or 'host'")
    check_fp64_supported(precision, beta, rng)
    p.reserved = 1 if rng == "host" else 0
    p.max_iter = int(nmf_kwargs.get("max_iter", 1000))
    p.tol = float(nmf_kwargs.get("tol", 1e-4))
    p.l1_reg_W = n_features * alpha_W * l1_ratio
    p.l1_reg_H = n_samples * alpha_H * l1_ratio
    p.l2_reg_W = n_features * alpha_W * (1.0 - l1_ratio)
    p.l2_reg_H = n_samples * alpha_H * (1.0 - l1_ratio)
    p.beta_loss = loss
    return p


def loss_code(beta):
    table = {"frobenius": LOSS_FROBENIUS, 2: LOSS_FROBENIUS, "kullback-leibler": LOSS_KULLBACK_LEIBLER,
             1: LOSS_KULLBACK_LEIBLER, "itakura-saito": LOSS_ITAKURA_SAITO, 0: LOSS_ITAKURA_SAITO}
    try:
        return table[beta]
    except (KeyError, TypeError):
        raise NotImplementedError("cnmf_b200: beta_loss must be 'frobenius' (2), 'kullback-leibler' (1) or "
                                  "'itakura-saito' (0) on the CUDA path (got %r)" % (beta,))


class Engine:

    def __init__(self, device=0):
        self.lib = _lib.load()
        self._h = ctypes.c_void_p()
        check(self.lib.cnmf_create(ctypes.byref(self._h), int(device)))
        self.device = int(device)

    def close(self):
        if self._h:
            self.lib.cnmf_destroy(self._h)
            self._h = ctypes.c_void_p()

    def __del__(self):
        try:
            self.close()
        except Exception:
            pass

    @property
    def launch_count(self):
        return int(self.lib.cnmf_launch_count(self._h))

    def profile(self, on=True):
        check(self.lib.cnmf_profile_enable(self._h, 1 if on else 0))

    def profile_get(self, kernel_class=0):
        ms, n, fl = ctypes.c_double(), ctypes.c_longlong(), ctypes.c_double()
        check(self.lib.cnmf_profile_get_class(self._h, int(kernel_class), ctypes.byref(ms), ctypes.byref(n),
                                              ctypes.byref(fl)))
        return ms.value, int(n.value), fl.value

    def mem_info(self):
        v = [ctypes.c_longlong() for _ in range(3)]
        check(self.lib.cnmf_mem_info(self._h, *[ctypes.byref(x) for x in v]))
        return tuple(int(x.value) for x in v)

    def last_timing(self):
        v = [ctypes.c_double() for _ in range(4)]
        check(self.lib.cnmf_last_timing(self._h, *[ctypes.byref(x) for x in v]))
        return dict(zip(("rng_ms", "h2d_ms", "solve_ms", "d2h_ms"), [x.value for x in v]))

    def nndsvd_chunk_limit(self, max_restarts):
        check(self.lib.cnmf_nndsvd_chunk_limit(self._h, int(max_restarts)))

    def dataset(self, X, precision=_DEFAULT_PRECISION, stream=None):
        return Dataset(self, X, precision, stream)

    def sparse_dataset(self, X, precision=_DEFAULT_PRECISION, stream=None):
        if is_fp64(precision):
            raise NotImplementedError("cnmf_b200: precision='fp64' needs a dense dataset; sparse (CSC) datasets hold "
                                      "float32 values")
        import scipy.sparse as sp
        C = sp.csc_matrix(X, dtype=np.float32)
        if not C.has_canonical_format:
            C = C.copy()
            C.sum_duplicates()
        n, g = C.shape
        col_ptr = np.ascontiguousarray(C.indptr, dtype=np.int64)
        row_idx = np.ascontiguousarray(C.indices, dtype=np.int32)
        vals = np.ascontiguousarray(C.data, dtype=np.float32)
        out = ctypes.c_void_p()
        check(self.lib.cnmf_dataset_create_csc(self._h, n, g, int(col_ptr[-1]), ptr(col_ptr), ptr(row_idx), ptr(vals),
                                               precision_code(precision), stream, ctypes.byref(out)))
        return Dataset(self, None, precision, _handle=out, sparse=True)

    def dense_dataset_bytes(self, n_rows, n_cols, precision=_DEFAULT_PRECISION):
        peak = ctypes.c_longlong()
        check(self.lib.cnmf_dataset_dense_bytes(int(n_rows), int(n_cols), precision_code(precision), ctypes.byref(peak)))
        return int(peak.value)

    def gemm_abt(self, A, B, precision=PRECISION_TF32X3, splits=1, reps=1, b_exact=False, k_scale=None,
                 out_col_scale=None):
        A, B = f32c(A), f32c(B)
        M, Kd = A.shape
        N = B.shape[0]
        assert B.shape[1] == Kd
        ks = None if k_scale is None else f32c(k_scale)
        cs = None if out_col_scale is None else f32c(out_col_scale)
        assert ks is None or ks.shape == (Kd,)
        assert cs is None or cs.shape == (N,)
        C = np.empty((M, N), np.float32)
        ms = ctypes.c_float(0)
        pc = precision_code(precision)
        pc = PRECISION_TF32X3 if pc == PRECISION_TF32X3_GENERAL else pc
        check(self.lib.cnmf_gemm_abt_host(self._h, pc, ptr(A), ptr(B), M, N, Kd, splits, 1 if b_exact else 0,
                                          ptr(ks), ptr(cs), ptr(C), reps, ctypes.byref(ms), None))
        return C, float(ms.value)

    def update_step(self, ks, rids, done, n, F, num, gram_in, solver="mu", pieces=None, gram=None, want_scalar=False,
                    cpb_tiles=1, l1=0.0, l2=0.0, piece_scale=None, pieces_hi=None, pieces_lo=None, tile_scale=None,
                    gram_out=None, scal_out=None):
        ks = np.ascontiguousarray(ks, np.int32)
        rids = np.ascontiguousarray(rids, np.int32)
        done = np.ascontiguousarray(done, np.int32)
        F = f32c(F).copy()
        SK, ld = F.shape
        assert SK == int(ks.sum()) and ld == -(-int(n) // 32) * 32
        num = f32c(num).reshape(-1, SK, ld) if num is not None else None
        gram_in = np.ascontiguousarray(gram_in, np.float64)
        n_rids = len(done)
        assert gram_in.shape == (n_rids, 32, 32)
        pmode = {None: _lib.UNIT_PIECES_NONE, "tf32": _lib.UNIT_PIECES_TF32, "f16": _lib.UNIT_PIECES_F16}[pieces]
        gmode = {None: _lib.UNIT_GRAM_NONE, "fused": _lib.UNIT_GRAM_FUSED, "standalone": _lib.UNIT_GRAM_STANDALONE}[gram]
        smode = {None: _lib.UNIT_SOLVER_NONE, "mu": SOLVER_MU, "cd": SOLVER_CD}[solver]
        pdt = np.float16 if pieces == "f16" else np.float32
        hi = lo = ts = None
        if pieces is not None:
            hi = np.zeros((SK, ld), pdt) if pieces_hi is None else np.ascontiguousarray(pieces_hi, pdt).copy()
            lo = np.zeros((SK, ld), pdt) if pieces_lo is None else np.ascontiguousarray(pieces_lo, pdt).copy()
        if pieces == "f16":
            nt = (ld + 511) // 512
            ts = np.zeros((SK, nt), np.float32) if tile_scale is None else f32c(tile_scale).copy()
        g_out = np.zeros((n_rids, 32, 32)) if gram_out is None else np.ascontiguousarray(gram_out, np.float64).copy()
        s_out = np.zeros(n_rids) if scal_out is None else np.ascontiguousarray(scal_out, np.float64).copy()
        ps = None if piece_scale is None else f32c(piece_scale)
        assert ps is None or ps.shape == (ld,)
        a = _lib.UpdateStepArgs()
        a.n_slots, a.n_rids, a.n, a.cpb_tiles = len(ks), n_rids, int(n), int(cpb_tiles)
        a.ks, a.rids, a.done = ptr(ks), ptr(rids), ptr(done)
        a.solver, a.pieces, a.gram, a.want_scalar = smode, pmode, gmode, 1 if want_scalar else 0
        a.nsplit = 1 if num is None else num.shape[0]
        a.l1, a.l2 = float(l1), float(l2)
        a.F, a.num, a.gram_in, a.piece_scale = ptr(F), ptr(num), ptr(gram_in), ptr(ps)
        a.pieces_hi, a.pieces_lo, a.tile_scale = ptr(hi), ptr(lo), ptr(ts)
        a.gram_out, a.scal_out = ptr(g_out), ptr(s_out)
        check(self.lib.cnmf_update_step_host(self._h, ctypes.byref(a), None))
        return dict(F=F, hi=hi, lo=lo, tile_scale=ts, gram=g_out, scal=s_out)

    def beta_step(self, ks, rids, done, side, loss, D, F_own, F_other, n_items, n_contract, op="update", l1=0.0, l2=0.0,
                  last=None, totals=None):
        ks = np.ascontiguousarray(ks, np.int32)
        rids = np.ascontiguousarray(rids, np.int32)
        done = np.ascontiguousarray(done, np.int32)
        SK, n_rids = int(ks.sum()), len(done)
        ld_i, ld_k = -(-int(n_items) // 32) * 32, -(-int(n_contract) // 32) * 32
        D = f32c(D)
        F = f32c(F_own).copy()
        Fo = f32c(F_other)
        assert D.shape == (n_contract, ld_i) and F.shape == (SK, ld_i) and Fo.shape == (SK, ld_k)
        lcode = {"kullback-leibler": LOSS_KULLBACK_LEIBLER, "itakura-saito": LOSS_ITAKURA_SAITO,
                 "frobenius": LOSS_FROBENIUS}[loss]
        oth = np.zeros(SK)
        lo = np.zeros(n_rids) if last is None else np.ascontiguousarray(last, np.float64).copy()
        tt = np.zeros((n_rids, 2)) if totals is None else np.ascontiguousarray(totals, np.float64).copy()
        assert lo.shape == (n_rids,) and tt.shape == (n_rids, 2)
        a = _lib.BetaStepArgs()
        a.n_slots, a.n_rids = len(ks), n_rids
        a.ks, a.rids, a.done = ptr(ks), ptr(rids), ptr(done)
        a.op = {"update": _lib.UNIT_BETA_UPDATE, "divergence": _lib.UNIT_BETA_DIVERGENCE}[op]
        a.side = {"W": _lib.UNIT_SIDE_W, "H": _lib.UNIT_SIDE_H}[side]
        a.loss, a.n_items, a.n_contract = lcode, int(n_items), int(n_contract)
        a.l1, a.l2 = float(l1), float(l2)
        a.D, a.F_own, a.F_other = ptr(D), ptr(F), ptr(Fo)
        a.oth_sum, a.last, a.totals = ptr(oth), ptr(lo), ptr(tt)
        check(self.lib.cnmf_beta_step_host(self._h, ctypes.byref(a), None))
        return dict(F=F, oth_sum=oth, last=lo, totals=tt)


class Dataset:

    def __init__(self, engine, X, precision=_DEFAULT_PRECISION, stream=None, _handle=None, sparse=False):
        self.engine = engine
        self.lib = engine.lib
        self.precision = precision_code(precision)
        self.fp64 = self.precision == PRECISION_FP64
        self.sparse = sparse
        self._d = ctypes.c_void_p()
        if _handle is not None:
            self._d = _handle
        else:
            if hasattr(X, "toarray"):
                X = X.toarray()
            if self.fp64:
                X = f64c(X)
                n, g = X.shape
                check(self.lib.cnmf_dataset_create_f64(engine._h, ptr(X), n, g, g, 0, stream, ctypes.byref(self._d)))
            else:
                X = f32c(X)
                n, g = X.shape
                check(self.lib.cnmf_dataset_create(engine._h, ptr(X), n, g, g, 0, self.precision, stream,
                                                   ctypes.byref(self._d)))
        n, g = ctypes.c_int(), ctypes.c_int()
        check(self.lib.cnmf_dataset_shape(self._d, ctypes.byref(n), ctypes.byref(g)))
        self.shape = (n.value, g.value)

    def close(self):
        if self._d:
            self.lib.cnmf_dataset_destroy(self._d)
            self._d = ctypes.c_void_p()

    def __del__(self):
        try:
            self.close()
        except Exception:
            pass

    def ld(self):
        a, b = ctypes.c_int(), ctypes.c_int()
        check(self.lib.cnmf_dataset_ld(self._d, ctypes.byref(a), ctypes.byref(b)))
        return a.value, b.value

    def solve_bytes_per_row(self):
        return int(self.lib.cnmf_solve_bytes_per_row(self._d))

    def max_rows_per_solve(self, fraction=0.8):
        free, _, cached = self.engine.mem_info()
        return max(1, int(fraction * (free + cached)) // max(1, self.solve_bytes_per_row()))

    def random_init_dev(self, ks, seeds, Wt_ptr, H_ptr):
        ks = np.ascontiguousarray(ks, dtype=np.int32)
        seeds = np.ascontiguousarray(seeds, dtype=np.uint32)
        check(self.lib.cnmf_random_init_dev(self._d, len(ks), ptr(ks), ptr(seeds), ctypes.c_void_p(Wt_ptr),
                                            ctypes.c_void_p(H_ptr), None))

    def nndsvd_init_dev(self, ks, seeds, init, Wt_ptr, H_ptr):
        ks = np.ascontiguousarray(ks, dtype=np.int32)
        seeds = np.ascontiguousarray(seeds, dtype=np.uint32)
        code = init_code(init, ks, *self.shape)
        if code == _lib.INIT_RANDOM:
            raise ValueError("nndsvd_init_dev: init=%r is the random init (random_init_dev)" % (init,))
        check(self.lib.cnmf_nndsvd_init_dev(self._d, len(ks), ptr(ks), ptr(seeds), code, ctypes.c_void_p(Wt_ptr),
                                            ctypes.c_void_p(H_ptr), None))

    def nndsvd_gemm(self, A, to_genes):
        A = np.ascontiguousarray(A, dtype=np.float64)
        n, g = self.shape
        assert A.shape[1] == (n if to_genes else g)
        C = np.empty((A.shape[0], g if to_genes else n))
        check(self.lib.cnmf_nndsvd_gemm_host(self._d, 1 if to_genes else 0, A.shape[0], ptr(A), ptr(C), None))
        return C

    def _init_params(self, ks, nmf_kwargs):
        p = self.params(nmf_kwargs)
        p.reserved |= init_code(nmf_kwargs.get("init", "random"), ks, *self.shape) << 1
        return p

    def factorize_seeds_dev(self, ks, seeds, out_ptr, ld_out, nmf_kwargs):
        ks = np.ascontiguousarray(ks, dtype=np.int32)
        seeds = np.ascontiguousarray(seeds, dtype=np.uint32)
        R = len(ks)
        p = self._init_params(ks, nmf_kwargs)
        self._check_loss(p)
        n_iter = np.zeros(R, np.int32)
        err = np.zeros(R, np.float64)
        check(self.lib.cnmf_factorize_seeds_dev(self._d, R, ptr(ks), ptr(seeds), ctypes.byref(p), ctypes.c_void_p(out_ptr),
                                                int(ld_out), ptr(n_iter), ptr(err), None))
        return n_iter, err

    def factorize_dev(self, ks, Wt0_ptr, H0_ptr, out_ptr, nmf_kwargs):
        ks = np.ascontiguousarray(ks, dtype=np.int32)
        R = len(ks)
        p = self.params(nmf_kwargs)
        self._check_loss(p)
        n_iter = np.zeros(R, np.int32)
        err = np.zeros(R, np.float64)
        check(self.lib.cnmf_factorize_dev(self._d, R, ptr(ks), ctypes.c_void_p(Wt0_ptr), ctypes.c_void_p(H0_ptr),
                                          ctypes.byref(p), ctypes.c_void_p(out_ptr), ptr(n_iter), ptr(err), None))
        return n_iter, err

    @property
    def exact(self):
        return bool(self.lib.cnmf_dataset_is_exact(self._d))

    @property
    def f16(self):
        return self.lib.cnmf_dataset_is_exact(self._d) == 2

    def min(self):
        m = ctypes.c_float()
        check(self.lib.cnmf_dataset_min(self._d, ctypes.byref(m), None))
        return float(m.value)

    def _check_loss(self, p):
        if p.beta_loss == LOSS_ITAKURA_SAITO and self.min() == 0:
            raise ValueError("When beta_loss <= 0 and X contains zeros, the solver may diverge. Please add small values "
                             "to X, or use a positive beta_loss.")

    def sums(self):
        s, q = ctypes.c_double(), ctypes.c_double()
        check(self.lib.cnmf_dataset_sums(self._d, ctypes.byref(s), ctypes.byref(q)))
        return s.value, q.value

    def col_stats(self, row_scale=None):
        g = self.shape[1]
        mean, var = np.empty(g), np.empty(g)
        if row_scale is None:
            check(self.lib.cnmf_dataset_col_stats(self._d, ptr(mean), ptr(var), None))
        else:
            rs = np.ascontiguousarray(row_scale, dtype=np.float64)
            assert rs.shape == (self.shape[0],)
            check(self.lib.cnmf_dataset_scaled_col_stats(self._d, ptr(rs), ptr(mean), ptr(var), None))
        return mean, var

    def row_sums(self):
        out = np.empty(self.shape[0])
        check(self.lib.cnmf_dataset_row_sums(self._d, ptr(out), None))
        return out

    def tpm_stats(self, target_sum=1e6):
        n, g = self.shape
        totals, mean, var = np.empty(n), np.empty(g), np.empty(g)
        check(self.lib.cnmf_dataset_tpm_stats(self._d, float(target_sum), ptr(totals), ptr(mean), ptr(var), None))
        return totals, mean, var

    def scale_rows(self, row_scale):
        rs = f32c(row_scale)
        assert rs.shape == (self.shape[0],)
        out = ctypes.c_void_p()
        check(self.lib.cnmf_dataset_scale_rows(self._d, ptr(rs), None, ctypes.byref(out)))
        return Dataset(self.engine, None, self.precision, _handle=out)

    def from_columns(self, cols, scale):
        cols = np.ascontiguousarray(cols, dtype=np.int32)
        scale = f32c(scale)
        out = ctypes.c_void_p()
        check(self.lib.cnmf_dataset_from_columns(self._d, ptr(cols), ptr(scale), len(cols), None, ctypes.byref(out)))
        return Dataset(self.engine, None, self.precision, _handle=out)

    def from_columns_div(self, cols, divisor):
        cols = np.ascontiguousarray(cols, dtype=np.int32)
        div = f64c(divisor)
        assert div.shape == cols.shape
        out = ctypes.c_void_p()
        check(self.lib.cnmf_dataset_from_columns_f64(self._d, ptr(cols), ptr(div), len(cols), None, ctypes.byref(out)))
        return Dataset(self.engine, None, self.precision, _handle=out)

    def params(self, nmf_kwargs):
        return make_params(nmf_kwargs, self.shape[0], self.shape[1], self.precision)

    def factorize(self, ks, seeds, nmf_kwargs, return_usages=False, W0=None, H0=None, X_host=None):
        ks = np.ascontiguousarray(ks, dtype=np.int32)
        R = len(ks)
        SK = int(ks.sum())
        n, g = self.shape
        p = self.params(nmf_kwargs)
        self._check_loss(p)
        dt = np.float64 if self.fp64 else np.float32
        spectra = np.empty((SK, g), dt)
        usages = np.empty((SK, n), dt) if return_usages else None
        n_iter = np.zeros(R, np.int32)
        err = np.zeros(R, np.float64)
        init = nmf_kwargs.get("init", "random")
        if W0 is None and init != "random" and X_host is not None:
            W0, H0 = nndsvd_starts(X_host, ks, seeds, init, dtype=dt)
        if self.fp64:
            if W0 is None:
                p.reserved |= init_code(init, ks, n, g) << 1
                seeds = np.ascontiguousarray(seeds, dtype=np.uint32)
                check(self.lib.cnmf_factorize_f64(self._d, R, ptr(ks), ptr(seeds), ctypes.byref(p), ptr(spectra),
                                                  ptr(usages), ptr(n_iter), ptr(err), None))
            else:
                W0, H0 = f64c(W0), f64c(H0)
                assert W0.shape == (SK, n) and H0.shape == (SK, g)
                check(self.lib.cnmf_factorize_init_f64(self._d, R, ptr(ks), ptr(W0), ptr(H0), ctypes.byref(p),
                                                       ptr(spectra), ptr(usages), ptr(n_iter), ptr(err), None))
        elif W0 is None:
            p.reserved |= init_code(init, ks, n, g) << 1
            seeds = np.ascontiguousarray(seeds, dtype=np.uint32)
            check(self.lib.cnmf_factorize(self._d, R, ptr(ks), ptr(seeds), ctypes.byref(p), ptr(spectra), ptr(usages),
                                          ptr(n_iter), ptr(err), None))
        else:
            W0, H0 = f32c(W0), f32c(H0)
            assert W0.shape == (SK, n) and H0.shape == (SK, g)
            check(self.lib.cnmf_factorize_init(self._d, R, ptr(ks), ptr(W0), ptr(H0), ctypes.byref(p), ptr(spectra),
                                               ptr(usages), ptr(n_iter), ptr(err), None))
        offs = np.concatenate([[0], np.cumsum(ks)])
        sp = [spectra[offs[r]:offs[r + 1]] for r in range(R)]
        us = [usages[offs[r]:offs[r + 1]].T for r in range(R)] if return_usages else None
        return sp, us, n_iter, err

    def refit(self, fixed, nmf_kwargs, transposed=False):
        fixed = f64c(fixed) if self.fp64 else f32c(fixed)
        k = fixed.shape[0]
        n, g = self.shape
        n_r, n_c = (g, n) if transposed else (n, g)
        assert fixed.shape[1] == n_c
        p = make_params(nmf_kwargs, n_r, n_c, self.precision, for_refit=True)
        self._check_loss(p)
        out = np.empty((n_r, k), fixed.dtype)
        it = ctypes.c_int32(0)
        err = ctypes.c_double(0)
        fn = self.lib.cnmf_refit_f64 if self.fp64 else self.lib.cnmf_refit
        check(fn(self._d, 1 if transposed else 0, k, ptr(fixed), ctypes.byref(p), ptr(out), ctypes.byref(it),
                 ctypes.byref(err), None))
        return out, int(it.value), float(err.value)

    def project_rows(self, Ut):
        Ut = f64c(Ut) if self.fp64 else f32c(Ut)
        k = Ut.shape[0]
        assert Ut.shape[1] == self.shape[0]
        out = np.empty((k, self.shape[1]), Ut.dtype)
        fn = self.lib.cnmf_project_rows_f64 if self.fp64 else self.lib.cnmf_project_rows
        check(fn(self._d, k, ptr(Ut), ptr(out), None))
        return out
```

include/cnmf_b200.h:

```cpp
#ifndef CNMF_B200_H
#define CNMF_B200_H

#include <stdint.h>

#ifdef __cplusplus
extern "C" {
#endif

#define CNMF_B200_ABI_VERSION 14
#define CNMF_MAX_COMPONENTS 32

typedef struct cnmf_handle_s* cnmf_handle_t;
typedef struct cnmf_dataset_s* cnmf_dataset_t;

enum { CNMF_SOLVER_MU = 0, CNMF_SOLVER_CD = 1 };
enum { CNMF_PRECISION_FP32 = 0, CNMF_PRECISION_TF32X3 = 1, CNMF_PRECISION_TF32X3_GENERAL = 2,
       CNMF_PRECISION_F16X2 = 3,
       CNMF_PRECISION_FP64 = 4 };

enum { CNMF_LOSS_FROBENIUS = 0, CNMF_LOSS_KULLBACK_LEIBLER = 1, CNMF_LOSS_ITAKURA_SAITO = 2 };

enum { CNMF_INIT_RANDOM = 0, CNMF_INIT_NNDSVD = 1, CNMF_INIT_NNDSVDA = 2, CNMF_INIT_NNDSVDAR = 3 };

typedef struct cnmf_nmf_params {
  int32_t solver;
  int32_t precision;
  int32_t max_iter;
  int32_t reserved;
  double tol;
  double l1_reg_W, l2_reg_W, l1_reg_H, l2_reg_H;
  int32_t beta_loss;
  int32_t reserved2;
} cnmf_nmf_params;

int cnmf_abi_version(void);
const char* cnmf_last_error(void);
int cnmf_create(cnmf_handle_t* out, int device);
int cnmf_destroy(cnmf_handle_t h);
long long cnmf_launch_count(cnmf_handle_t h);
int cnmf_mem_info(cnmf_handle_t h, long long* free_bytes, long long* total_bytes, long long* cached_bytes);
long long cnmf_solve_bytes_per_row(cnmf_dataset_t d);

int cnmf_profile_enable(cnmf_handle_t h, int on);
int cnmf_profile_get(cnmf_handle_t h, double* gemm_ms, long long* gemm_launches, double* gemm_flops);
int cnmf_profile_get_class(cnmf_handle_t h, int kernel_class, double* ms, long long* launches, double* work);

int cnmf_last_timing(cnmf_handle_t h, double* rng_ms, double* h2d_ms, double* solve_ms, double* d2h_ms);

int cnmf_dataset_create(cnmf_handle_t h, const float* X, int n_rows, int n_cols, long long ld,
                        int src_is_device, int precision, void* stream, cnmf_dataset_t* out);
int cnmf_dataset_create_csc(cnmf_handle_t h, int n_rows, int n_cols, long long nnz, const int64_t* col_ptr,
                            const int32_t* row_idx, const float* values, int precision, void* stream,
                            cnmf_dataset_t* out);
int cnmf_dataset_dense_bytes(int n_rows, int n_cols, int precision, long long* peak);
int cnmf_dataset_from_columns(cnmf_dataset_t src, const int32_t* cols_host, const float* col_scale_host,
                              int n_cols, void* stream, cnmf_dataset_t* out);
int cnmf_dataset_destroy(cnmf_dataset_t d);
int cnmf_dataset_shape(cnmf_dataset_t d, int* n_rows, int* n_cols);
int cnmf_dataset_ld(cnmf_dataset_t d, int* ld_rows, int* ld_cols);
int cnmf_dataset_sums(cnmf_dataset_t d, double* sum, double* sum_sq);
int cnmf_dataset_min(cnmf_dataset_t d, float* min_host, void* stream);
int cnmf_dataset_is_exact(cnmf_dataset_t d);
int cnmf_dataset_col_stats(cnmf_dataset_t d, double* mean_host, double* var_host, void* stream);

int cnmf_dataset_row_sums(cnmf_dataset_t d, double* row_sums_host, void* stream);
int cnmf_dataset_scaled_col_stats(cnmf_dataset_t d, const double* row_scale_host, double* mean_host, double* var_host,
                                  void* stream);
int cnmf_dataset_tpm_stats(cnmf_dataset_t d, double target_sum, double* totals_host, double* mean_host,
                           double* var_host, void* stream);
int cnmf_dataset_scale_rows(cnmf_dataset_t src, const float* row_scale_host, void* stream, cnmf_dataset_t* out);

int cnmf_random_init_host(uint32_t seed, double avg, int n_samples, int n_features, int k,
                          float* Wt, long long ldW, float* H, long long ldH);

int cnmf_random_init_dev(cnmf_dataset_t d, int n_restarts, const int32_t* ks, const uint32_t* seeds, float* Wt_dev,
                         float* H_dev, void* stream);

int cnmf_nndsvd_init_dev(cnmf_dataset_t d, int n_restarts, const int32_t* ks, const uint32_t* seeds, int init,
                         float* Wt_dev, float* H_dev, void* stream);
int cnmf_nndsvd_chunk_limit(cnmf_handle_t h, int max_restarts);
int cnmf_nndsvd_gemm_host(cnmf_dataset_t d, int to_genes, int M, const double* A_host, double* C_host, void* stream);

int cnmf_dataset_create_f64(cnmf_handle_t h, const double* X, int n_rows, int n_cols, long long ld, int src_is_device,
                            void* stream, cnmf_dataset_t* out);
int cnmf_dataset_from_columns_f64(cnmf_dataset_t src, const int32_t* cols_host, const double* divisor_host, int n_cols,
                                  void* stream, cnmf_dataset_t* out);
int cnmf_factorize_f64(cnmf_dataset_t d, int n_restarts, const int32_t* ks, const uint32_t* seeds,
                       const cnmf_nmf_params* params, double* spectra_host, double* usages_host, int32_t* n_iter_host,
                       double* err_host, void* stream);
int cnmf_factorize_init_f64(cnmf_dataset_t d, int n_restarts, const int32_t* ks, const double* Wt0_host,
                            const double* H0_host, const cnmf_nmf_params* params, double* spectra_host,
                            double* usages_host, int32_t* n_iter_host, double* err_host, void* stream);
int cnmf_refit_f64(cnmf_dataset_t d, int transposed, int k, const double* fixed_host, const cnmf_nmf_params* params,
                   double* out_host, int32_t* n_iter_host, double* err_host, void* stream);
int cnmf_project_rows_f64(cnmf_dataset_t d, int k, const double* Ut_host, double* out_host, void* stream);

int cnmf_factorize(cnmf_dataset_t d, int n_restarts, const int32_t* ks, const uint32_t* seeds,
                   const cnmf_nmf_params* params, float* spectra_host, float* usages_host,
                   int32_t* n_iter_host, double* err_host, void* stream);

int cnmf_factorize_seeds_dev(cnmf_dataset_t d, int n_restarts, const int32_t* ks, const uint32_t* seeds,
                             const cnmf_nmf_params* params, float* spectra_dev, long long ld_out,
                             int32_t* n_iter_host, double* err_host, void* stream);

int cnmf_allgather_spectra(void* nccl_comm, const float* local_dev, long long rows_per_rank, long long ld,
                           float* merged_dev, void* stream);
int cnmf_comm_unique_id(char* id_out_128);
int cnmf_comm_create(cnmf_handle_t h, const char* id_128, int rank, int world, void** comm_out);
int cnmf_comm_destroy(void* nccl_comm);

int cnmf_factorize_init(cnmf_dataset_t d, int n_restarts, const int32_t* ks, const float* Wt0_host,
                        const float* H0_host, const cnmf_nmf_params* params, float* spectra_host,
                        float* usages_host, int32_t* n_iter_host, double* err_host, void* stream);

int cnmf_factorize_dev(cnmf_dataset_t d, int n_restarts, const int32_t* ks, const float* Wt0_dev,
                       const float* H0_dev, const cnmf_nmf_params* params, float* spectra_dev,
                       int32_t* n_iter_host, double* err_host, void* stream);

int cnmf_refit(cnmf_dataset_t d, int transposed, int k, const float* fixed_host, const cnmf_nmf_params* params,
               float* out_host, int32_t* n_iter_host, double* err_host, void* stream);

int cnmf_project_rows(cnmf_dataset_t d, int k, const float* Ut_host, float* out_host, void* stream);

int cnmf_gemm_abt_host(cnmf_handle_t h, int precision, const float* A, const float* B, int M, int N, int Kd,
                       int splits, int b_exact, const float* k_scale, const float* out_col_scale, float* C, int reps,
                       float* ms_out, void* stream);

enum { CNMF_UNIT_SOLVER_NONE = -1 };
enum { CNMF_UNIT_PIECES_NONE = 0, CNMF_UNIT_PIECES_TF32 = 1, CNMF_UNIT_PIECES_F16 = 2 };
enum { CNMF_UNIT_GRAM_NONE = 0, CNMF_UNIT_GRAM_FUSED = 1, CNMF_UNIT_GRAM_STANDALONE = 2 };
typedef struct cnmf_update_step_args {
  int32_t n_slots;
  int32_t n_rids;
  const int32_t* ks;
  const int32_t* rids;
  const int32_t* done;
  int32_t n;
  int32_t cpb_tiles;
  int32_t solver;
  int32_t pieces;
  int32_t gram;
  int32_t want_scalar;
  int32_t nsplit;
  float l1, l2;
  float* F;
  const float* num;
  const double* gram_in;
  const float* piece_scale;
  void* pieces_hi;
  void* pieces_lo;
  float* tile_scale;
  double* gram_out;
  double* scal_out;
} cnmf_update_step_args;
int cnmf_update_step_host(cnmf_handle_t h, const cnmf_update_step_args* args, void* stream);

enum { CNMF_UNIT_BETA_UPDATE = 0, CNMF_UNIT_BETA_DIVERGENCE = 1 };
enum { CNMF_UNIT_SIDE_W = 0, CNMF_UNIT_SIDE_H = 1 };
typedef struct cnmf_beta_step_args {
  int32_t n_slots;
  int32_t n_rids;
  const int32_t* ks;
  const int32_t* rids;
  const int32_t* done;
  int32_t op;
  int32_t side;
  int32_t loss;
  int32_t n_items, n_contract;
  float l1, l2;
  const float* D;
  float* F_own;
  const float* F_other;
  double* oth_sum;
  double* last;
  double* totals;
} cnmf_beta_step_args;
int cnmf_beta_step_host(cnmf_handle_t h, const cnmf_beta_step_args* args, void* stream);

int cnmf_l2_normalize_rows(cnmf_handle_t h, float* S_dev, int R, int G, int ld, void* stream);
int cnmf_local_density(cnmf_handle_t h, const float* S_dev, int R, int G, int ld, int n_neighbors,
                       float* density_dev, float* D_dev, void* stream);
int cnmf_col_stats_dev(cnmf_handle_t h, const float* S_dev, int R, int G, int ld, double* mean_host,
                       double* var_host, void* stream);
int cnmf_gather_rows(cnmf_handle_t h, const float* src_dev, int ld_src, const int32_t* idx_host, int n, int G,
                     float* dst_dev, int ld_dst, void* stream);
int cnmf_sq_dists_to_rows(cnmf_handle_t h, const float* S_dev, int R, int G, int ld, const int32_t* idx_host,
                          int n_c, float* out_host, void* stream);
int cnmf_kmeans_assign(cnmf_handle_t h, const float* S_dev, int R, int G, int ld, const float* centers_host, int K,
                       int32_t* labels_dev, double* sums_host, int32_t* counts_host, float* mind_dev,
                       int32_t* n_changed_host, double* inertia_host, void* stream);
int cnmf_kmeans_step(cnmf_handle_t h, const float* S_dev, int R, int G, int ld, int K, const float* C32_cur_dev,
                     const double* C64_cur_dev, double* C64_new_dev, float* C32_new_dev, int32_t* labels_dev,
                     float* mind_dev, double* sums_dev, int32_t* counts_dev, int32_t* n_changed_host,
                     int32_t* any_empty_host, double* shift_host, void* stream);
int cnmf_kmeans_fit(cnmf_handle_t h, const float* S_dev, int R, int G, int ld, int K, int n_init, int max_iter,
                    double tol_abs, const int32_t* first_idx_host, const double* uniforms_host, int n_trials,
                    int32_t* labels_host, double* inertia_host, int32_t* n_iter_host, int32_t* needs_host_path,
                    void* stream);
int cnmf_cluster_dist_sums(cnmf_handle_t h, const float* S_dev, int R, int G, int ld, const int32_t* labels_dev,
                           int K, double* sums_host, void* stream);
int cnmf_cluster_median(cnmf_handle_t h, const float* S_dev, int R, int G, int ld, const int32_t* labels_dev, int K,
                        float* M_dev, int ldm, void* stream);

int cnmf_l2_normalize_rows_f64(cnmf_handle_t h, double* S_dev, int R, int G, int ld, void* stream);
int cnmf_local_density_f64(cnmf_handle_t h, const double* S_dev, int R, int G, int ld, int n_neighbors,
                           double* density_dev, double* D_dev, void* stream);
int cnmf_col_stats_dev_f64(cnmf_handle_t h, const double* S_dev, int R, int G, int ld, double* mean_host,
                           double* var_host, void* stream);
int cnmf_gather_rows_f64(cnmf_handle_t h, const double* src_dev, int ld_src, const int32_t* idx_host, int n, int G,
                         double* dst_dev, int ld_dst, void* stream);
int cnmf_sq_dists_to_rows_f64(cnmf_handle_t h, const double* S_dev, int R, int G, int ld, const int32_t* idx_host,
                              int n_c, double* out_host, void* stream);
int cnmf_kmeans_assign_f64(cnmf_handle_t h, const double* S_dev, int R, int G, int ld, const double* centers_host,
                           int K, int32_t* labels_dev, double* sums_host, int32_t* counts_host, double* mind_dev,
                           int32_t* n_changed_host, double* inertia_host, void* stream);
int cnmf_kmeans_step_f64(cnmf_handle_t h, const double* S_dev, int R, int G, int ld, int K, const double* C64_cur_dev,
                         double* C64_new_dev, int32_t* labels_dev, double* mind_dev, double* sums_dev,
                         int32_t* counts_dev, int32_t* n_changed_host, int32_t* any_empty_host, double* shift_host,
                         void* stream);
int cnmf_kmeans_fit_f64(cnmf_handle_t h, const double* S_dev, int R, int G, int ld, int K, int n_init, int max_iter,
                        double tol_abs, const int32_t* first_idx_host, const double* uniforms_host, int n_trials,
                        int32_t* labels_host, double* inertia_host, int32_t* n_iter_host, int32_t* needs_host_path,
                        void* stream);
int cnmf_cluster_dist_sums_f64(cnmf_handle_t h, const double* S_dev, int R, int G, int ld, const int32_t* labels_dev,
                               int K, double* sums_host, void* stream);
int cnmf_cluster_median_f64(cnmf_handle_t h, const double* S_dev, int R, int G, int ld, const int32_t* labels_dev,
                            int K, double* M_dev, int ldm, void* stream);

#ifdef __cplusplus
}
#endif
#endif
```

Before: 547.0.

## Widen GEMM n-tiles to 168/192 for exact-B forms, fix BM at 128

Swaps the tall-M variant (three consumer warpgroups with BM=192) for a fixed BM=128 with wider n-tiles of 128, 168 or 192 columns in the exact-B tf32x3 and fp16 paths. A cost model picks the tile width from wave quantisation, and n_tiles is now computed from the padded column count. Wider tiles reuse each A tile across more columns and can cut partial waves, but they raise accumulator register pressure, so setmaxnreg goes to 232 for consumers and 40 for the producer. The gemm entry point also gains a tile_n override, which bumps the ABI version.

```diff
diff --git a/cnmf_b200/_lib.py b/cnmf_b200/_lib.py
--- a/cnmf_b200/_lib.py
+++ b/cnmf_b200/_lib.py
@@ -107,7 +107,7 @@
     "cnmf_factorize_dev": (_i, [_vp, _i, _vp, _vp, _vp, _pp(NmfParams), _vp, _vp, _vp, _vp]),
     "cnmf_refit": (_i, [_vp, _i, _i, _vp, _pp(NmfParams), _vp, _pp(_c.c_int32), _pp(_d), _vp]),
     "cnmf_project_rows": (_i, [_vp, _i, _vp, _vp, _vp]),
-    "cnmf_gemm_abt_host": (_i, [_vp, _i, _vp, _vp, _i, _i, _i, _i, _i, _vp, _vp, _vp, _i, _pp(_c.c_float), _vp]),
+    "cnmf_gemm_abt_host": (_i, [_vp, _i, _vp, _vp, _i, _i, _i, _i, _i, _vp, _vp, _i, _vp, _i, _pp(_c.c_float), _vp]),
     "cnmf_update_step_host": (_i, [_vp, _pp(UpdateStepArgs), _vp]),
     "cnmf_beta_step_host": (_i, [_vp, _pp(BetaStepArgs), _vp]),
     "cnmf_l2_normalize_rows": (_i, [_vp, _vp, _i, _i, _i, _vp]),
@@ -135,7 +135,7 @@
 _lib = None
 
 
-ABI_VERSION = 14
+ABI_VERSION = 15
 
 
 def load():
diff --git a/cnmf_b200/csrc/capi_refit.cu b/cnmf_b200/csrc/capi_refit.cu
--- a/cnmf_b200/csrc/capi_refit.cu
+++ b/cnmf_b200/csrc/capi_refit.cu
@@ -518,8 +518,8 @@
 }
 
 int cnmf_gemm_abt_host(cnmf_handle_t h, int precision, const float* A, const float* B, int M, int N, int Kd, int splits,
-                       int b_exact, const float* k_scale, const float* out_col_scale, float* C, int reps, float* ms_out,
-                       void* stream) {
+                       int b_exact, const float* k_scale, const float* out_col_scale, int tile_n, float* C, int reps,
+                       float* ms_out, void* stream) {
   CNMF_REQUIRE(h && A && B && C && M > 0 && N > 0 && Kd > 0, "gemm_abt_host: bad arguments");
   const bool f16 = precision == CNMF_PRECISION_F16X2;
   CNMF_REQUIRE(!b_exact || f16 || precision == CNMF_PRECISION_TF32X3, "gemm_abt_host: b_exact needs tf32x3 or f16x2");
@@ -567,6 +567,7 @@
   GemmArgs g{};
   g.M = M; g.N = N; g.Kd = Kd; g.lda = lda; g.ldb = lda; g.ldc = ldc;
   g.C = dC; g.c_split_stride = (long long)M * ldc; g.splits = splits; g.splits_effective = se;
+  g.tile_n = tile_n;
   const Operand Bop{dB, dBh, dBl, N, Kd, lda};
   cudaEvent_t e0, e1;
   CNMF_CUDA_CHECK(cudaEventCreate(&e0));
diff --git a/cnmf_b200/csrc/gemm.h b/cnmf_b200/csrc/gemm.h
--- a/cnmf_b200/csrc/gemm.h
+++ b/cnmf_b200/csrc/gemm.h
@@ -19,6 +19,7 @@
   int f16;
   const float* a_tile_scale;
   int a_tiles;
+  int tile_n;
 };
 
 int gemm_effective_splits(int Kd, int splits, int f16 = 0);
diff --git a/cnmf_b200/csrc/gemm_tf32x3.cu b/cnmf_b200/csrc/gemm_tf32x3.cu
--- a/cnmf_b200/csrc/gemm_tf32x3.cu
+++ b/cnmf_b200/csrc/gemm_tf32x3.cu
@@ -14,14 +14,12 @@
 
 namespace {
 
-constexpr int BN = 128;
+constexpr int BM = 128;
+constexpr int NUM_THREADS = 128 * (1 + BM / 64);
 constexpr int BK = 32;
 constexpr long long WAIT_TIMEOUT_CYCLES = 4000000000LL;
 
-template <int BM>
-constexpr int num_threads() { return 128 * (1 + BM / 64); }
-
-template <int BM, int STAGES, bool BEXACT>
+template <int BN, int STAGES, bool BEXACT>
 struct SmemLayout {
   static constexpr int A_BYTES = BM * BK * 4;
   static constexpr int B_BYTES = BN * BK * 4;
@@ -113,47 +111,41 @@
 template <int N>
 __device__ __forceinline__ void wgmma_wait() { asm volatile("wgmma.wait_group.sync.aligned %0;" ::"n"(N) : "memory"); }
 
-template <bool F16>
-__device__ __forceinline__ void wgmma_m64n128(float (&d)[64], uint64_t adesc, uint64_t bdesc, uint32_t acc) {
-  if constexpr (F16) {
-    asm volatile(
-      "{\n\t.reg .pred p;\n\t"
-      "setp.ne.b32 p, %66, 0;\n\t"
-      "wgmma.mma_async.sync.aligned.m64n128k16.f32.f16.f16 {"
-      "%0, %1, %2, %3, %4, %5, %6, %7, %8, %9, %10, %11, %12, %13, %14, %15, "
-      "%16, %17, %18, %19, %20, %21, %22, %23, %24, %25, %26, %27, %28, %29, %30, %31, "
-      "%32, %33, %34, %35, %36, %37, %38, %39, %40, %41, %42, %43, %44, %45, %46, %47, "
-      "%48, %49, %50, %51, %52, %53, %54, %55, %56, %57, %58, %59, %60, %61, %62, %63 "
-      "}, %64, %65, p, 1, 1, 0, 0;\n\t}"
-      : "+f"(d[0]), "+f"(d[1]), "+f"(d[2]), "+f"(d[3]), "+f"(d[4]), "+f"(d[5]), "+f"(d[6]), "+f"(d[7]),
-        "+f"(d[8]), "+f"(d[9]), "+f"(d[10]), "+f"(d[11]), "+f"(d[12]), "+f"(d[13]), "+f"(d[14]), "+f"(d[15]),
-        "+f"(d[16]), "+f"(d[17]), "+f"(d[18]), "+f"(d[19]), "+f"(d[20]), "+f"(d[21]), "+f"(d[22]), "+f"(d[23]),
-        "+f"(d[24]), "+f"(d[25]), "+f"(d[26]), "+f"(d[27]), "+f"(d[28]), "+f"(d[29]), "+f"(d[30]), "+f"(d[31]),
-        "+f"(d[32]), "+f"(d[33]), "+f"(d[34]), "+f"(d[35]), "+f"(d[36]), "+f"(d[37]), "+f"(d[38]), "+f"(d[39]),
-        "+f"(d[40]), "+f"(d[41]), "+f"(d[42]), "+f"(d[43]), "+f"(d[44]), "+f"(d[45]), "+f"(d[46]), "+f"(d[47]),
-        "+f"(d[48]), "+f"(d[49]), "+f"(d[50]), "+f"(d[51]), "+f"(d[52]), "+f"(d[53]), "+f"(d[54]), "+f"(d[55]),
-        "+f"(d[56]), "+f"(d[57]), "+f"(d[58]), "+f"(d[59]), "+f"(d[60]), "+f"(d[61]), "+f"(d[62]), "+f"(d[63])
-      : "l"(adesc), "l"(bdesc), "r"(acc));
-  } else {
-    asm volatile(
-      "{\n\t.reg .pred p;\n\t"
-      "setp.ne.b32 p, %66, 0;\n\t"
-      "wgmma.mma_async.sync.aligned.m64n128k8.f32.tf32.tf32 {"
-      "%0, %1, %2, %3, %4, %5, %6, %7, %8, %9, %10, %11, %12, %13, %14, %15, "
-      "%16, %17, %18, %19, %20, %21, %22, %23, %24, %25, %26, %27, %28, %29, %30, %31, "
-      "%32, %33, %34, %35, %36, %37, %38, %39, %40, %41, %42, %43, %44, %45, %46, %47, "
-      "%48, %49, %50, %51, %52, %53, %54, %55, %56, %57, %58, %59, %60, %61, %62, %63 "
-      "}, %64, %65, p, 1, 1;\n\t}"
-      : "+f"(d[0]), "+f"(d[1]), "+f"(d[2]), "+f"(d[3]), "+f"(d[4]), "+f"(d[5]), "+f"(d[6]), "+f"(d[7]),
-        "+f"(d[8]), "+f"(d[9]), "+f"(d[10]), "+f"(d[11]), "+f"(d[12]), "+f"(d[13]), "+f"(d[14]), "+f"(d[15]),
-        "+f"(d[16]), "+f"(d[17]), "+f"(d[18]), "+f"(d[19]), "+f"(d[20]), "+f"(d[21]), "+f"(d[22]), "+f"(d[23]),
-        "+f"(d[24]), "+f"(d[25]), "+f"(d[26]), "+f"(d[27]), "+f"(d[28]), "+f"(d[29]), "+f"(d[30]), "+f"(d[31]),
-        "+f"(d[32]), "+f"(d[33]), "+f"(d[34]), "+f"(d[35]), "+f"(d[36]), "+f"(d[37]), "+f"(d[38]), "+f"(d[39]),
-        "+f"(d[40]), "+f"(d[41]), "+f"(d[42]), "+f"(d[43]), "+f"(d[44]), "+f"(d[45]), "+f"(d[46]), "+f"(d[47]),
-        "+f"(d[48]), "+f"(d[49]), "+f"(d[50]), "+f"(d[51]), "+f"(d[52]), "+f"(d[53]), "+f"(d[54]), "+f"(d[55]),
-        "+f"(d[56]), "+f"(d[57]), "+f"(d[58]), "+f"(d[59]), "+f"(d[60]), "+f"(d[61]), "+f"(d[62]), "+f"(d[63])
-      : "l"(adesc), "l"(bdesc), "r"(acc));
-  }
+#define CNMF_R64                                                                      \
+  "%0, %1, %2, %3, %4, %5, %6, %7, %8, %9, %10, %11, %12, %13, %14, %15, "            \
+  "%16, %17, %18, %19, %20, %21, %22, %23, %24, %25, %26, %27, %28, %29, %30, %31, "  \
+  "%32, %33, %34, %35, %36, %37, %38, %39, %40, %41, %42, %43, %44, %45, %46, %47, "  \
+  "%48, %49, %50, %51, %52, %53, %54, %55, %56, %57, %58, %59, %60, %61, %62, %63"
+#define CNMF_R84 CNMF_R64 ", %64, %65, %66, %67, %68, %69, %70, %71, %72, %73, %74, %75, %76, %77, %78, %79, " \
+  "%80, %81, %82, %83"
+#define CNMF_R96 CNMF_R84 ", %84, %85, %86, %87, %88, %89, %90, %91, %92, %93, %94, %95"
+#define CNMF_D4(i) "+f"(d[i]), "+f"(d[i + 1]), "+f"(d[i + 2]), "+f"(d[i + 3])
+#define CNMF_D8(i) CNMF_D4(i), CNMF_D4(i + 4)
+#define CNMF_D64 CNMF_D8(0), CNMF_D8(8), CNMF_D8(16), CNMF_D8(24), CNMF_D8(32), CNMF_D8(40), CNMF_D8(48), CNMF_D8(56)
+#define CNMF_D84 CNMF_D64, CNMF_D8(64), CNMF_D8(72), CNMF_D4(80)
+#define CNMF_D96 CNMF_D64, CNMF_D8(64), CNMF_D8(72), CNMF_D8(80), CNMF_D8(88)
+#define CNMF_WGMMA(N, REGS, IA, IB, IACC, ...)                                                                        \
+  template <bool F16>                                                                                                 \
+  __device__ __forceinline__ void wgmma_m64n##N(float (&d)[N / 2], uint64_t adesc, uint64_t bdesc, uint32_t acc) {    \
+    if constexpr (F16)                                                                                                \
+      asm volatile("{\n\t.reg .pred p;\n\tsetp.ne.b32 p, %" IACC ", 0;\n\t"                                          \
+                   "wgmma.mma_async.sync.aligned.m64n" #N "k16.f32.f16.f16 {" REGS "}, %" IA ", %" IB                 \
+                   ", p, 1, 1, 0, 0;\n\t}"                                                                            \
+                   : __VA_ARGS__ : "l"(adesc), "l"(bdesc), "r"(acc));                                                 \
+    else                                                                                                              \
+      asm volatile("{\n\t.reg .pred p;\n\tsetp.ne.b32 p, %" IACC ", 0;\n\t"                                          \
+                   "wgmma.mma_async.sync.aligned.m64n" #N "k8.f32.tf32.tf32 {" REGS "}, %" IA ", %" IB ", p, 1, 1;\n\t}" \
+                   : __VA_ARGS__ : "l"(adesc), "l"(bdesc), "r"(acc));                                                 \
+  }
+CNMF_WGMMA(128, CNMF_R64, "64", "65", "66", CNMF_D64)
+CNMF_WGMMA(168, CNMF_R84, "84", "85", "86", CNMF_D84)
+CNMF_WGMMA(192, CNMF_R96, "96", "97", "98", CNMF_D96)
+
+template <int BN, bool F16>
+__device__ __forceinline__ void wgmma_tile(float (&d)[BN / 2], uint64_t adesc, uint64_t bdesc, uint32_t acc) {
+  if constexpr (BN == 128) wgmma_m64n128<F16>(d, adesc, bdesc, acc);
+  else if constexpr (BN == 168) wgmma_m64n168<F16>(d, adesc, bdesc, acc);
+  else wgmma_m64n192<F16>(d, adesc, bdesc, acc);
 }
 
 struct TileOrder {
@@ -174,18 +166,18 @@
   np = o.group_n ? q : p;
 }
 
-template <int BM, int STAGES, bool BEXACT, bool F16>
+template <int BN, int STAGES, bool BEXACT, bool F16>
 __device__ __forceinline__ void
 gemm_body(const CUtensorMap& tmA_hi, const CUtensorMap& tmA_lo, const CUtensorMap& tmB_hi, const CUtensorMap& tmB_lo,
           float* __restrict__ C, int M, int ldc, long long c_split_stride,
           const TileOrder& ord, int n_tiles, int splits, int total_kb, int kb_per_split, int chain_kb,
           const float* __restrict__ out_scale, const float* __restrict__ a_tile_scale, int a_tiles, int a_gshift) {
   static_assert(!F16 || BEXACT, "the fp16 path exists for exact integer B operands only");
-  static_assert(BM == 128 || BM == 192, "two or three consumer warpgroups");
+  static_assert(BN == 128 || (BEXACT && (BN == 168 || BN == 192)), "wide n-tiles in the exact-B forms only");
   constexpr int NC = BM / 64;
   constexpr int BKE = F16 ? 2 * BK : BK;
   constexpr int KSTEP_BYTES = 32;
-  using L = SmemLayout<BM, STAGES, BEXACT>;
+  using L = SmemLayout<BN, STAGES, BEXACT>;
   extern __shared__ uint8_t smem_raw[];
   const uint32_t smem_base = (smem_u32(smem_raw) + 1023u) & ~1023u;
 
@@ -211,9 +203,9 @@
 
   const int items = ord.m_tiles * ord.n_pairs * splits;
 
-  constexpr bool REBALANCE = NC == 3;
+  constexpr bool REBALANCE = BN > 128;
   if (wg == 0) {
-    if constexpr (REBALANCE) setmaxnreg_dec<32>();
+    if constexpr (REBALANCE) setmaxnreg_dec<40>();
     if (threadIdx.x == 0) {
       int stage = 0;
       uint32_t phase = 0;
@@ -245,7 +237,7 @@
       }
     }
   } else {
-    if constexpr (REBALANCE) setmaxnreg_inc<160>();
+    if constexpr (REBALANCE) setmaxnreg_inc<232>();
     constexpr uint32_t TURN_BAR = 1, TURN_THREADS = 256;
     const int cw = wg - 1;
     const uint32_t a_off = static_cast<uint32_t>(cw * 64 * 128);
@@ -260,14 +252,14 @@
       const int kb0 = z * kb_per_split;
       const int kb1 = min(total_kb, kb0 + kb_per_split);
       const int row0 = mt * BM + cw * 64 + warp * 16 + (lane >> 2);
-      float acc[64];
-#pragma unroll
-      for (int i = 0; i < 64; ++i) acc[i] = 0.f;
+      float acc[BN / 2];
+#pragma unroll
+      for (int i = 0; i < BN / 2; ++i) acc[i] = 0.f;
       const float* sc_row0 = (F16 && a_tile_scale && row0 < M) ? a_tile_scale + static_cast<long long>(row0) * a_tiles : nullptr;
       const float* sc_row1 = (F16 && a_tile_scale && row0 + 8 < M) ? a_tile_scale + static_cast<long long>(row0 + 8) * a_tiles : nullptr;
       for (int c0 = kb0; c0 < kb1; c0 += chain_kb) {
         const int c1 = min(kb1, c0 + chain_kb);
-        float d[64];
+        float d[BN / 2];
         int prev = -1;
         for (int kb = c0; kb < c1; ++kb) {
           mbar_wait<false>(full_bar(stage), phase);
@@ -282,9 +274,9 @@
           for (int k = 0; k < BK * 4 / KSTEP_BYTES; ++k) {
             const uint64_t koff = static_cast<uint64_t>((k * KSTEP_BYTES) >> 4);
             const uint32_t acc0 = (kb > c0 || k > 0) ? 1u : 0u;
-            wgmma_m64n128<F16>(d, a_lo + koff, b_hi + koff, acc0);
-            if constexpr (!BEXACT) wgmma_m64n128<F16>(d, a_hi + koff, b_lo + koff, 1u);
-            wgmma_m64n128<F16>(d, a_hi + koff, b_hi + koff, 1u);
+            wgmma_tile<BN, F16>(d, a_lo + koff, b_hi + koff, acc0);
+            if constexpr (!BEXACT) wgmma_tile<BN, F16>(d, a_hi + koff, b_lo + koff, 1u);
+            wgmma_tile<BN, F16>(d, a_hi + koff, b_hi + koff, 1u);
           }
           wgmma_commit();
           named_bar_arrive(next_bar, TURN_THREADS);
@@ -301,7 +293,7 @@
           const float s0 = sc_row0 ? sc_row0[c0 >> a_gshift] : 1.f;
           const float s1 = sc_row1 ? sc_row1[c0 >> a_gshift] : 1.f;
 #pragma unroll
-          for (int i = 0; i < 64; i += 4) {
+          for (int i = 0; i < BN / 2; i += 4) {
             acc[i] = fmaf(d[i], s0, acc[i]);
             acc[i + 1] = fmaf(d[i + 1], s0, acc[i + 1]);
             acc[i + 2] = fmaf(d[i + 2], s1, acc[i + 2]);
@@ -309,15 +301,16 @@
           }
         } else {
 #pragma unroll
-          for (int i = 0; i < 64; ++i) acc[i] += d[i];
+          for (int i = 0; i < BN / 2; ++i) acc[i] += d[i];
         }
       }
       if (nt >= n_tiles) continue;
-      constexpr int EPI_J = 8;
+      constexpr int EPI_J = (BN / 8) % 8 == 0 ? 8 : 7;
+      static_assert((BN / 8) % EPI_J == 0, "column groups in whole batches");
       float* cbase = C + static_cast<long long>(z) * c_split_stride;
       const int colq = nt * BN + 2 * (lane & 3);
 #pragma unroll
-      for (int j0 = 0; j0 < 16; j0 += EPI_J) {
+      for (int j0 = 0; j0 < BN / 8; j0 += EPI_J) {
         float2 sc[EPI_J];
 #pragma unroll
         for (int j = 0; j < EPI_J; ++j) {
@@ -343,14 +336,14 @@
   cluster_sync();
 }
 
-template <int BM, int STAGES, bool BEXACT, bool F16>
-__global__ void __cluster_dims__(2, 1, 1) __launch_bounds__(num_threads<BM>(), 1)
+template <int BN, int STAGES, bool BEXACT, bool F16>
+__global__ void __cluster_dims__(2, 1, 1) __launch_bounds__(NUM_THREADS, 1)
 gemm_tf32x3_kernel(const __grid_constant__ CUtensorMap tmA_hi, const __grid_constant__ CUtensorMap tmA_lo,
                    const __grid_constant__ CUtensorMap tmB_hi, const __grid_constant__ CUtensorMap tmB_lo,
                    float* __restrict__ C, int M, int ldc, long long c_split_stride,
                    const TileOrder ord, int n_tiles, int splits, int total_kb, int kb_per_split, int chain_kb,
                    const float* __restrict__ out_scale, const float* __restrict__ a_tile_scale, int a_tiles, int a_gshift) {
-  gemm_body<BM, STAGES, BEXACT, F16>(tmA_hi, tmA_lo, tmB_hi, tmB_lo, C, M, ldc, c_split_stride, ord, n_tiles, splits,
+  gemm_body<BN, STAGES, BEXACT, F16>(tmA_hi, tmA_lo, tmB_hi, tmB_lo, C, M, ldc, c_split_stride, ord, n_tiles, splits,
                                      total_kb, kb_per_split, chain_kb, out_scale, a_tile_scale, a_tiles, a_gshift);
 }
 
@@ -432,10 +425,9 @@
   return best;
 }
 
-template <int BM, int STAGES, bool BEXACT, bool F16>
+template <int BN, int STAGES, bool BEXACT, bool F16>
 int launch(const GemmArgs& g, cudaStream_t stream) {
-  using L = SmemLayout<BM, STAGES, BEXACT>;
-  constexpr int NUM_THREADS = num_threads<BM>();
+  using L = SmemLayout<BN, STAGES, BEXACT>;
   constexpr int BKE = F16 ? 2 * BK : BK;
   CUtensorMap mAh, mAl, mBh, mBl;
   int rc;
@@ -447,7 +439,7 @@
   CNMF_CUDA_CHECK(cudaGetDevice(&dev));
   CNMF_CUDA_CHECK(cudaDeviceGetAttribute(&l2, cudaDevAttrL2CacheSize, dev));
   const int m_tiles = (g.M + BM - 1) / BM;
-  const int n_tiles = (g.N + BN - 1) / BN;
+  const int n_tiles = (std::min(g.ldc, (g.N + 31) / 32 * 32) + BN - 1) / BN;
   const int n_pairs = (n_tiles + 1) / 2;
   const int total_kb = (g.Kd + BKE - 1) / BKE;
   int splits = g.splits < 1 ? 1 : g.splits;
@@ -457,7 +449,7 @@
   splits = (total_kb + kb_per_split - 1) / kb_per_split;
   if (splits != g.splits_effective) { set_last_error("gemm: splits_effective mismatch (use gemm_effective_splits)"); return -1; }
 
-  auto kern = gemm_tf32x3_kernel<BM, STAGES, BEXACT, F16>;
+  auto kern = gemm_tf32x3_kernel<BN, STAGES, BEXACT, F16>;
   static int max_clusters[64] = {};
   int clusters_cap = dev >= 0 && dev < 64 ? max_clusters[dev] : 0;
   if (clusters_cap == 0) {
@@ -501,6 +493,28 @@
   return (total_kb + kb_per_split - 1) / kb_per_split;
 }
 
+static int pick_tile_n(const GemmArgs& g) {
+  if (!g.b_exact) return 128;
+  int dev = 0, sms = 0;
+  CNMF_CUDA_CHECK(cudaGetDevice(&dev));
+  CNMF_CUDA_CHECK(cudaDeviceGetAttribute(&sms, cudaDevAttrMultiProcessorCount, dev));
+  const long long pairs = std::max(1, sms / 2);
+  const long long m_items = static_cast<long long>((g.M + BM - 1) / BM) * g.splits_effective;
+  const int cols = std::min(g.ldc, (g.N + 31) / 32 * 32);
+  auto cost = [&](int bn, int per_item) {
+    const long long items = m_items * (((cols + bn - 1) / bn + 1) / 2);
+    return (items + pairs - 1) / pairs * per_item;
+  };
+  const long long narrow = cost(128, 100);
+  int best = 128;
+  long long best_cost = narrow * 98 / 100;
+  for (const auto& [bn, per_item] : {std::pair<int, int>{168, 125}, std::pair<int, int>{192, 142}}) {
+    const long long c = cost(bn, per_item);
+    if (c <= best_cost) { best_cost = c; best = bn; }
+  }
+  return best;
+}
+
 int gemm_tf32x3(const GemmArgs& g, cudaStream_t stream) {
   CNMF_REQUIRE(g.M > 0 && g.N > 0 && g.Kd > 0, "gemm: empty problem");
   CNMF_REQUIRE(g.lda % 4 == 0 && g.ldb % 4 == 0 && g.ldc % 4 == 0, "gemm: leading dimensions must be multiples of 4 floats");
@@ -508,14 +522,22 @@
                 reinterpret_cast<uintptr_t>(g.B_hi) | reinterpret_cast<uintptr_t>(g.B_lo) |
                 reinterpret_cast<uintptr_t>(g.C) | reinterpret_cast<uintptr_t>(g.out_col_scale)) % 16 == 0,
                "gemm: pointers must be 16-byte aligned");
-  const bool tall = g.splits_effective > 1 && g.M >= 2048;
+  CNMF_REQUIRE(g.tile_n == 0 || g.tile_n == 128 || (g.b_exact && (g.tile_n == 168 || g.tile_n == 192)),
+               "gemm: tile_n must be 0 (the launcher's choice), 128, or 168 / 192 with an exact B");
+  const int bn = g.tile_n ? g.tile_n : pick_tile_n(g);
   if (g.f16) {
     CNMF_REQUIRE(g.b_exact, "gemm: the fp16 path needs an exact B operand");
     CNMF_REQUIRE(g.lda % 8 == 0 && g.ldb % 8 == 0, "gemm: fp16 leading dimensions must be multiples of 8 halves");
     CNMF_REQUIRE(!g.a_tile_scale || g.a_tiles * 512 >= g.Kd, "gemm: a_tiles does not cover the reduction length");
-    return tall ? launch<192, 3, true, true>(g, stream) : launch<128, 4, true, true>(g, stream);
-  }
-  if (g.b_exact) return tall ? launch<192, 3, true, false>(g, stream) : launch<128, 4, true, false>(g, stream);
+    if (bn == 168) return launch<168, 4, true, true>(g, stream);
+    if (bn == 192) return launch<192, 4, true, true>(g, stream);
+    return launch<128, 4, true, true>(g, stream);
+  }
+  if (g.b_exact) {
+    if (bn == 168) return launch<168, 4, true, false>(g, stream);
+    if (bn == 192) return launch<192, 4, true, false>(g, stream);
+    return launch<128, 4, true, false>(g, stream);
+  }
   return launch<128, 3, false, false>(g, stream);
 }
 
diff --git a/cnmf_b200/engine.py b/cnmf_b200/engine.py
--- a/cnmf_b200/engine.py
+++ b/cnmf_b200/engine.py
@@ -200,7 +200,7 @@
         return int(peak.value)
 
     def gemm_abt(self, A, B, precision=PRECISION_TF32X3, splits=1, reps=1, b_exact=False, k_scale=None,
-                 out_col_scale=None):
+                 out_col_scale=None, tile_n=0):
         A, B = f32c(A), f32c(B)
         M, Kd = A.shape
         N = B.shape[0]
@@ -214,7 +214,7 @@
         pc = precision_code(precision)
         pc = PRECISION_TF32X3 if pc == PRECISION_TF32X3_GENERAL else pc
         check(self.lib.cnmf_gemm_abt_host(self._h, pc, ptr(A), ptr(B), M, N, Kd, splits, 1 if b_exact else 0,
-                                          ptr(ks), ptr(cs), ptr(C), reps, ctypes.byref(ms), None))
+                                          ptr(ks), ptr(cs), int(tile_n), ptr(C), reps, ctypes.byref(ms), None))
         return C, float(ms.value)
 
     def update_step(self, ks, rids, done, n, F, num, gram_in, solver="mu", pieces=None, gram=None, want_scalar=False,
diff --git a/include/cnmf_b200.h b/include/cnmf_b200.h
--- a/include/cnmf_b200.h
+++ b/include/cnmf_b200.h
@@ -7,7 +7,7 @@
 extern "C" {
 #endif
 
-#define CNMF_B200_ABI_VERSION 14
+#define CNMF_B200_ABI_VERSION 15
 #define CNMF_MAX_COMPONENTS 32
 
 typedef struct cnmf_handle_s* cnmf_handle_t;
@@ -123,8 +123,8 @@
 int cnmf_project_rows(cnmf_dataset_t d, int k, const float* Ut_host, float* out_host, void* stream);
 
 int cnmf_gemm_abt_host(cnmf_handle_t h, int precision, const float* A, const float* B, int M, int N, int Kd,
-                       int splits, int b_exact, const float* k_scale, const float* out_col_scale, float* C, int reps,
-                       float* ms_out, void* stream);
+                       int splits, int b_exact, const float* k_scale, const float* out_col_scale, int tile_n, float* C,
+                       int reps, float* ms_out, void* stream);
 
 enum { CNMF_UNIT_SOLVER_NONE = -1 };
 enum { CNMF_UNIT_PIECES_NONE = 0, CNMF_UNIT_PIECES_TF32 = 1, CNMF_UNIT_PIECES_F16 = 2 };
```

Result: faster. 576.0, median of 6 (+5.3%).
